# cvg/limap

Hardware: AMD Instinct MI355X
Metric: 3D line candidates scored/sec (100 views x 500 segs per GPU, matched topk=10) (higher is better)
Workload: dtype f64

## Files before the change

### limap_amd/csrc/lt_api.cpp

```cpp

#include "lt_host.h"

using namespace lt;
using namespace lt_impl;

namespace lt_trace {
typedef int (*push_fn)(const char *);
typedef int (*pop_fn)(void);
static push_fn g_push = nullptr;
static pop_fn g_pop = nullptr;
static void init_once() {
  static bool done = false;
  if (done) return;
  done = true;
  const char *sw = getenv("LT_ROCTX");
  if (sw && sw[0] == '0') return;
  const char *libs[] = {"librocprofiler-sdk-roctx.so.1", "librocprofiler-sdk-roctx.so", "libroctx64.so.4", "libroctx64.so"};
  for (const char *l : libs) {
    void *h = dlopen(l, RTLD_LAZY | RTLD_GLOBAL);
    if (!h) continue;
    g_push = (push_fn)dlsym(h, "roctxRangePushA");
    g_pop = (pop_fn)dlsym(h, "roctxRangePop");
    if (g_push && g_pop) return;
    g_push = nullptr;
// ... 204 lines not shown

double now_ms() {
  return std::chrono::duration<double, std::milli>(std::chrono::steady_clock::now().time_since_epoch()).count();
}

}

namespace lt_impl {

double multiplier(double score_th) { return 1.0 / std::sqrt(-std::log(score_th) * 2.0); }

LinkCfg2 make_l2(const lt_config &c) {
  LinkCfg2 l;
  l.score_th = c.l2_score_th; l.th_angle = c.l2_th_angle; l.th_overlap = c.l2_th_overlap;
  l.th_smartoverlap = c.l2_th_smartoverlap; l.th_smartangle = c.l2_th_smartangle;
  l.th_perp = c.l2_th_perp; l.th_innerseg = c.l2_th_innerseg;
  l.mult = multiplier(c.l2_score_th);
  l.use_angle = c.l2_use_angle; l.use_overlap = c.l2_use_overlap; l.use_smartangle = c.l2_use_smartangle;
  l.use_perp = c.l2_use_perp; l.use_innerseg = c.l2_use_innerseg; l.pad_ = 0;
  return l;
}
LinkCfg3 make_l3(const lt_config &c) {
  LinkCfg3 l;
  l.score_th = c.l3_score_th; l.th_angle = c.l3_th_angle; l.th_overlap = c.l3_th_overlap;
  l.th_smartoverlap = c.l3_th_smartoverlap; l.th_smartangle = c.l3_th_smartangle;
  l.th_perp = c.l3_th_perp; l.th_innerseg = c.l3_th_innerseg; l.th_scaleinv = c.l3_th_scaleinv;
  l.mult = multiplier(c.l3_score_th);
  l.use_angle = c.l3_use_angle; l.use_overlap = c.l3_use_overlap; l.use_smartangle = c.l3_use_smartangle;
  l.use_perp = c.l3_use_perp; l.use_innerseg = c.l3_use_innerseg; l.use_scaleinv = c.l3_use_scaleinv;
  return l;
}

GenCfg make_gen(const lt_ctx *ctx) {
  const lt_config &c = ctx->cfg;
  GenCfg g;
  g.min_length_2d = c.min_length_2d; g.angle_th = c.line_tri_angle_threshold; g.iou_th = c.IoU_threshold;
  g.sens_th = c.sensitivity_threshold; g.var2d = c.var2d;
  for (int k = 0; k < 3; ++k) { g.lo[k] = ctx->lo[k]; g.hi[k] = ctx->hi[k]; }
  g.use_ranges = ctx->ranges_on; g.use_endpoints = c.use_endpoints_triangulation;
  g.disable_algebraic = c.disable_algebraic_triangulation;
  g.force_undecided = test_switch("LT_TEST_NO_FAST_GATES") != nullptr;
  if (c.use_vp && !c.disable_vp_triangulation) g.force_undecided = 1;
  double th = c.line_tri_angle_threshold;
  if (th > 1e-3 && th < 89.0) {
    double s = std::sin(th * kPi / 180.0);
    g.sin_lo = s * (1.0 - 1e-7);
    g.sin_hi = s * (1.0 + 1e-7);
  } else {
    g.sin_lo = -1.0;
    g.sin_hi = 1e300;
  }
  {
    const double ths = c.sensitivity_threshold;
    if (ths > 1e-3 && ths < 89.0) {
      const double sn = std::sin(ths * kPi / 180.0);
      g.sens_lo = sn * (1.0 - 1e-7);
      g.sens_hi = sn * (1.0 + 1e-7);
      g.sens_lo2 = g.sens_lo * g.sens_lo * (1.0 - 1e-9);
      g.sens_hi2 = g.sens_hi * g.sens_hi * (1.0 + 1e-9);
    } else {
      g.sens_lo = -1.0;
      g.sens_hi = 1e300;
      g.sens_lo2 = -1.0;
      g.sens_hi2 = 1e300;
    }
    if (test_switch("LT_TEST_NO_FAST_GATES")) {
      g.sens_lo2 = -1.0;
      g.sens_hi2 = 1e300;
    }
  }
  const double L = c.min_length_2d;
  if (L > 0.0) {
    g.len_lo2 = L * L * (1.0 - 1e-12);
    g.len_hi2 = L * L * (1.0 + 1e-12);
  } else if (L == 0.0) {
    g.len_lo2 = g.len_hi2 = 0.0;
  } else {
    g.len_lo2 = g.len_hi2 = -1.0;
  }
  return g;
}

ScoreCfg make_score(const lt_ctx *ctx) {
  ScoreCfg s;
  s.l2 = make_l2(ctx->cfg);
  s.l3 = make_l3(ctx->cfg);
  s.l3.use_angle = 1; s.l3.use_overlap = 0; s.l3.use_perp = 0; s.l3.use_innerseg = 0; s.l3.use_scaleinv = 1;
  double th = s.l3.th_angle * (1.0 + 1e-6) + 1e-6;
  s.cos_guard = (th < 90.0) ? std::cos(th * kPi / 180.0) : -1.0;
  if (test_switch("LT_TEST_NO_SCORE_GUARDS")) s.cos_guard = -1.0;
  s.fullscore_th = ctx->cfg.fullscore_th;
  s.max_valid_conns = ctx->cfg.max_valid_conns;
  auto band = [](double th, double *lo, double *hi) -> bool {
    if (!(th >= 1e-3 && th <= 0.999)) {
      *lo = -1.0;
      *hi = 1e300;
      return false;
    }
    const double q = std::sqrt(-2.0 * std::log(th));
    *lo = q * (1.0 - 1e-9);
    *hi = q * (1.0 + 1e-9);
    return true;
  };
  const bool b3 = band(s.l3.score_th, &s.q3_lo, &s.q3_hi), b2 = band(s.l2.score_th, &s.q2_lo, &s.q2_hi);
  const bool pos = s.l3.th_angle > 0.0 && s.l3.th_scaleinv > 0.0 && s.l2.th_angle > 0.0 && s.l2.th_perp > 0.0 &&
                   s.l2.th_smartangle > 0.0 && s.l2.th_smartangle <= s.l2.th_angle && s.l2.th_smartoverlap > s.l2.th_overlap;
  s.fast = (b3 && b2 && pos && !s.l2.use_innerseg && !test_switch("LT_TEST_PAIR_SCORE_TERMS")) ? 1 : 0;
  return s;
}

int bits_for(long long n) {
  int b = 1;
  while (b < 32 && (1ll << b) < n) ++b;
  return b;
}

int init_common(lt_ctx *ctx, int n_img, const int32_t *img_ids, const int64_t *seg_off_in,
                const std::vector<int> &perm) {
  ctx->n_img = n_img;
  ctx->img_ids.resize(n_img);
  ctx->id2idx.clear();
  ctx->seg_off.assign(n_img + 1, 0);
  for (int i = 0; i < n_img; ++i) {
    ctx->img_ids[i] = img_ids[perm[i]];
    if (ctx->id2idx.count(ctx->img_ids[i])) return fail(ctx, LT_ERR_ARGUMENT, "duplicate image id in Init");
    ctx->id2idx[ctx->img_ids[i]] = i;
    long long m = seg_off_in[perm[i] + 1] - seg_off_in[perm[i]];
    if (m < 0) return fail(ctx, LT_ERR_ARGUMENT, "seg_off must be non-decreasing");
    if (m > 65535) return fail(ctx, LT_ERR_ARGUMENT, "more than 65535 lines in one image (uint16 line ids, util/types.h:16)");
    ctx->seg_off[i + 1] = ctx->seg_off[i] + m;
  }
  ctx->G = ctx->seg_off[n_img];
  if (ctx->G >= (1ll << 32) - 1) return fail(ctx, LT_ERR_ARGUMENT, "too many nodes (>= 2^32-1)");
  ctx->h_node_img.resize(ctx->G);
  for (int i = 0; i < n_img; ++i)
    for (long long g = ctx->seg_off[i]; g < ctx->seg_off[i + 1]; ++g) ctx->h_node_img[g] = i;
  ctx->triangulated.assign(n_img, 0);
  ctx->neighbors.assign(n_img, {});
  lt_host::host_block_release(ctx->best_c_blk);
  ctx->best_c_blk = lt_host::host_block_acquire(sizeof(Cand) * (size_t)std::max<long long>(ctx->G, 1));
  ctx->best_c = (Cand *)ctx->best_c_blk.p;
  if (!ctx->best_c) return fail(ctx, LT_ERR_RUNTIME, "out of host memory for the per-node results");
  ctx->best_c_set.assign(n_img, 0);
  ctx->best_score.assign(ctx->G, 0.0);
  ctx->best_src2.assign(2 * ctx->G, 0);
  ctx->n_tris.assign(ctx->G, 0);
  ctx->has_best.assign(ctx->G, 0);
  ctx->valid_edges.reset(ctx->G);
  ctx->dbg_pool.clear(); ctx->dbg_off.assign((size_t)ctx->G, 0); ctx->dbg_cnt.assign((size_t)ctx->G, 0);
  ctx->vp_ready = false;
  ctx->pts_ready = false; ctx->sfm_given = false; ctx->pts_dirty = false;
  ctx->h_seg_pts.clear(); ctx->h_seg_pt_off.clear(); ctx->h_sfm_ids.clear(); ctx->h_sfm_xyz.clear();
  ctx->tracks.clear();
  ctx->tracks_done = false;
  ctx->job_mode = 0;
  ctx->job_imgs.clear(); ctx->job_nbs.clear(); ctx->job_order.clear();
  ctx->h_m_off.assign(1, 0); ctx->h_m_pairs.clear(); ctx->streamed_ints = 0;
  ctx->h_c_off.clear(); ctx->h_ovf_off.clear(); ctx->h_line0.clear(); ctx->h_ovf.clear();
  ctx->rows_sorted = true;
  ctx->uploaded = ctx->ran = ctx->downloaded = false;
  return LT_OK;
}

int build_invariants(lt_ctx *ctx, const double *hk = nullptr, const double *hq = nullptr, const double *ht = nullptr,
                     const double *hs = nullptr, bool sync = true) {
  hipStream_t st = ctx->stream;
  ENSURE(ctx, ctx->d_cams, sizeof(Cam) * (size_t)std::max(ctx->n_img, 1));
  ENSURE(ctx, ctx->d_segs, sizeof(Seg) * (size_t)std::max<long long>(ctx->G, 1));
  ENSURE(ctx, ctx->d_seg_off, sizeof(long long) * (size_t)(ctx->n_img + 1));
  ENSURE(ctx, ctx->d_node_img, sizeof(int) * (size_t)std::max<long long>(ctx->G, 1));
  HIPCHK(ctx, hipMemcpyAsync(ctx->d_seg_off.p, ctx->seg_off.data(), sizeof(long long) * (ctx->n_img + 1),
                             hipMemcpyHostToDevice, st));
  if (ctx->G > 0)
    HIPCHK(ctx, hipMemcpyAsync(ctx->d_node_img.p, ctx->h_node_img.data(), sizeof(int) * ctx->G,
                               hipMemcpyHostToDevice, st));
  launch_build_cams(st, ctx->n_img, ctx->d_kvec.as<double>(), ctx->d_qvec.as<double>(), ctx->d_tvec.as<double>(),
                    ctx->d_cams.as<Cam>());
  ENSURE(ctx, ctx->d_seg_gates, seg_gate_bytes() * (size_t)std::max<long long>(ctx->G, 1));
  launch_build_segs(st, ctx->G, ctx->n_img, ctx->d_seg_off.as<long long>(), ctx->d_segs_raw.as<double>(),
                    ctx->cfg.add_halfpix ? 0.5 : 0.0, ctx->d_cams.as<Cam>(), ctx->d_segs.as<Seg>(), ctx->d_seg_gates.p);
  HIPCHK(ctx, hipGetLastError());
  if (sync) HIPCHK(ctx, hipStreamSynchronize(st));
  {
    const int n = ctx->n_img;
    std::vector<double> k(4 * (size_t)n), q(4 * (size_t)n), t(3 * (size_t)n);
    if (hk && hq && ht && hs) {
      std::memcpy(k.data(), hk, 32 * (size_t)n);
      std::memcpy(q.data(), hq, 32 * (size_t)n);
      std::memcpy(t.data(), ht, 24 * (size_t)n);
      std::vector<double>().swap(ctx->h_segs);
      ctx->h_segs_ptr = hs;
      ctx->h_segs_add = ctx->cfg.add_halfpix ? 0.5 : 0.0;
    } else {
      ctx->h_segs.assign(4 * (size_t)ctx->G, 0.0);
      if (n > 0) {
        HIPCHK(ctx, hipMemcpy(k.data(), ctx->d_kvec.p, 32 * (size_t)n, hipMemcpyDeviceToHost));
        HIPCHK(ctx, hipMemcpy(q.data(), ctx->d_qvec.p, 32 * (size_t)n, hipMemcpyDeviceToHost));
        HIPCHK(ctx, hipMemcpy(t.data(), ctx->d_tvec.p, 24 * (size_t)n, hipMemcpyDeviceToHost));
      }
      if (ctx->G > 0)
        HIPCHK(ctx, hipMemcpy(ctx->h_segs.data(), ctx->d_segs_raw.p, 32 * (size_t)ctx->G, hipMemcpyDeviceToHost));
    }
    if (!(hk && hq && ht && hs)) {
      ctx->h_segs_ptr = ctx->h_segs.data();
      ctx->h_segs_add = ctx->cfg.add_halfpix ? 0.5 : 0.0;
    }
    ctx->h_cams.resize(n);
    for (int i = 0; i < n; ++i) cam_build(&k[4 * i], &q[4 * i], &t[3 * i], &ctx->h_cams[i]);
  }
  ctx->inited = true;
  return LT_OK;
}

void build_job_tables(lt_ctx *ctx) {
  const int n_img = ctx->n_img;
  ctx->h_nb_off.assign(n_img + 1, 0);
  std::vector<int> job_pos(n_img, -1);
  for (size_t j = 0; j < ctx->job_imgs.size(); ++j) job_pos[ctx->job_imgs[j]] = (int)j;
  ctx->h_blk_img.clear(); ctx->h_blk_nb.clear(); ctx->h_blk_slot.clear(); ctx->h_blk_order.clear();
  ctx->max_nb = 1;
  for (int i = 0; i < n_img; ++i) {
    ctx->h_nb_off[i] = (long long)ctx->h_blk_img.size();
    int j = job_pos[i];
    if (j < 0) continue;
    const auto &nbs = ctx->job_nbs[j];
    ctx->max_nb = std::max(ctx->max_nb, (int)nbs.size());
    for (size_t k = 0; k < nbs.size(); ++k) {
      ctx->h_blk_img.push_back(i);
      ctx->h_blk_nb.push_back(nbs[k]);
      ctx->h_blk_slot.push_back((int)k);
      ctx->h_blk_order.push_back(ctx->job_order[j][k]);
    }
  }
  ctx->h_nb_off[n_img] = (long long)ctx->h_blk_img.size();
  ctx->n_blk = (int)ctx->h_blk_img.size();
  ctx->h_blk_line_base.assign(ctx->n_blk + 1, 0);
  ctx->max_nb_segs = 0;
  ctx->max_own_segs = 0;
  for (int b = 0; b < ctx->n_blk; ++b) {
    int i1 = ctx->h_blk_img[b];
    int i2 = ctx->h_blk_nb[b];
    ctx->max_nb_segs = std::max(ctx->max_nb_segs, (int)(ctx->seg_off[i2 + 1] - ctx->seg_off[i2]));
    ctx->max_own_segs = std::max(ctx->max_own_segs, (int)(ctx->seg_off[i1 + 1] - ctx->seg_off[i1]));
    ctx->h_blk_line_base[b + 1] = ctx->h_blk_line_base[b] + (ctx->seg_off[i1 + 1] - ctx->seg_off[i1]) + 1;
  }
}

}

extern "C" {

void lt_config_default(lt_config *c) {
  std::memset(c, 0, sizeof(*c));
  c->min_length_2d = 20.0; c->line_tri_angle_threshold = 5.0; c->IoU_threshold = 0.1;
  c->sensitivity_threshold = 70.0; c->var2d = 2.0;
  c->fullscore_th = 1.0; c->max_valid_conns = 1000; c->min_num_outer_edges = 1;
  c->merging_strategy = 0; c->num_outliers_aggregator = 2;
  c->l2_score_th = 0.5; c->l2_th_angle = 8.0; c->l2_th_overlap = 0.1; c->l2_th_smartoverlap = 0.2;
  c->l2_th_smartangle = 1.0; c->l2_th_perp = 5.0; c->l2_th_innerseg = 5.0;
  c->l2_use_angle = 1; c->l2_use_overlap = 1; c->l2_use_smartangle = 1; c->l2_use_perp = 1; c->l2_use_innerseg = 0;
  c->l3_score_th = 0.5; c->l3_th_angle = 10.0; c->l3_th_overlap = 0.01; c->l3_th_smartoverlap = 0.1;
  c->l3_th_smartangle = 1.0; c->l3_th_perp = 0.02; c->l3_th_innerseg = 0.02; c->l3_th_scaleinv = 0.01;
  c->l3_use_angle = 1; c->l3_use_overlap = 1; c->l3_use_smartangle = 1; c->l3_use_perp = 0;
  c->l3_use_innerseg = 1; c->l3_use_scaleinv = 0;
}

int lt_abi_version(void) { return 2; }
uint64_t lt_sizeof_config(void) { return (uint64_t)sizeof(lt_config); }

lt_ctx *lt_create(const lt_config *cfg, int device) {
  int n_dev = 0;
  hipError_t e = hipGetDeviceCount(&n_dev);
  if (e != hipSuccess || n_dev <= 0) {
    std::fprintf(stderr, "limap_amd: no HIP device available (%s); this backend has no CPU fallback\n",
                 hipGetErrorString(e));
    return nullptr;
  }
  if (device < 0 || device >= n_dev) {
    std::fprintf(stderr, "limap_amd: device %d out of range (%d devices)\n", device, n_dev);
    return nullptr;
  }
  if (hipSetDevice(device) != hipSuccess) return nullptr;
  lt_ctx *ctx = new lt_ctx();
  ctx->cfg = *cfg;
  ctx->device = device;
  if (!lt_host::stream_set_acquire(device, &ctx->stream, ctx->ev)) {
    if (hipStreamCreateWithFlags(&ctx->stream, hipStreamNonBlocking) != hipSuccess) {
      delete ctx;
      return nullptr;
    }
    for (auto &ev : ctx->ev) (void)hipEventCreate(&ev);
  }
  ctx->pool_stream = ctx->stream;
  ctx->h_pinned_blk = lt_host::host_block_acquire(4096);
  ctx->h_pinned = ctx->h_pinned_blk.pinned ? (long long *)ctx->h_pinned_blk.p : nullptr;
  return ctx;
}

void lt_destroy(lt_ctx *ctx) {
  if (!ctx) return;
  (void)finish_run(ctx);
  (void)hipSetDevice(ctx->device);
  (void)hipStreamSynchronize(ctx->stream);
  DevBuf *bufs[] = {&ctx->d_kvec, &ctx->d_qvec, &ctx->d_tvec, &ctx->d_segs_raw, &ctx->d_cams, &ctx->d_segs,
                    &ctx->d_seg_off, &ctx->d_node_img, &ctx->d_nb_off, &ctx->d_blk_img, &ctx->d_blk_nb,
                    &ctx->d_blk_slot, &ctx->d_blk_order, &ctx->d_m_off, &ctx->d_m_pairs, &ctx->d_c_stream, &ctx->d_ovf, &ctx->d_rowdesc, &ctx->d_pairs,
                    &ctx->d_keys, &ctx->d_rows, &ctx->d_row_blk, &ctx->d_skeys, &ctx->d_srows, &ctx->d_sort_tmp,
                    &ctx->d_conn_off, &ctx->d_st_c, &ctx->d_st_l, &ctx->d_flags, &ctx->d_pos, &ctx->d_scan_tmp,
                    &ctx->d_item_off, &ctx->d_masks, &ctx->d_mask_cnt, &ctx->d_mask_pos, &ctx->d_cand, &ctx->d_hcand, &ctx->d_hlite,
                    &ctx->d_rm_line, &ctx->d_rm_act, &ctx->d_rm_edges, &ctx->d_rm_cnt,
                    &ctx->d_lite, &ctx->d_tri_off, &ctx->d_score, &ctx->d_best_idx, &ctx->d_edge_flag,
                    &ctx->d_nvalid, &ctx->d_edge_off, &ctx->d_edges, &ctx->d_best_c, &ctx->d_best_score,
                    &ctx->d_best_src, &ctx->d_ntris, &ctx->d_err, &ctx->d_blk_line_base, &ctx->d_cnt_bl,
                    &ctx->d_st_key, &ctx->d_wave_count, &ctx->d_wave_pos, &ctx->d_ntris_u, &ctx->d_cand_node,
                    &ctx->d_pair_counter, &ctx->d_result3, &ctx->d_tile_order, &ctx->d_scan_status, &ctx->d_perm, &ctx->d_rng, &ctx->d_chunks, &ctx->d_cand_meta, &ctx->d_st_row, &ctx->d_surv_count, &ctx->d_seg_gates, &ctx->d_blkrec, &ctx->d_seg_vp, &ctx->d_seg_has_vp, &ctx->d_base_bl, &ctx->d_blk_chunk_off, &ctx->d_needed, &ctx->d_seg_pts, &ctx->d_seg_pt_off, &ctx->d_sfm_xyz,
                    &ctx->d_place_perm, &ctx->d_ex_rec, &ctx->d_ex_ent, &ctx->d_node_rec, &ctx->d_ex_z, &ctx->d_tile_list, &ctx->d_tail_keys, &ctx->d_tail_skeys, &ctx->d_tail_sims, &ctx->d_tail_mark,
                    &ctx->d_tail_pos, &ctx->d_tail_recs, &ctx->d_tail_nodes, &ctx->d_tail_tmp, &ctx->d_tail_keep,
                    &ctx->d_tail_kpos, &ctx->d_sp_slots, &ctx->d_sp_cnt, &ctx->d_sp_ovf, &ctx->d_sp_pairs, &ctx->d_sp_desc,
                    &ctx->d_run_len, &ctx->d_slot_row0, &ctx->d_blk_nruns, &ctx->d_ln_flag, &ctx->d_blk_surv, &ctx->d_blk_rnd0,
                    &ctx->d_round_count};
  lt_host::host_block_release(ctx->h_pinned_blk);
  if (ctx->tail_pend.active) lt_host::host_block_release(ctx->tail_pend.hb);
  if (ctx->ev_tail) (void)hipEventDestroy(ctx->ev_tail);
  lt_host::host_block_release(ctx->best_c_blk);
  lt_host::host_block_release(ctx->init_blk);
  for (DevBuf *b : bufs) b->release();
  for (auto &e : ctx->ev_b)
    if (e) (void)hipEventDestroy(e);
  for (auto &e : ctx->ev_end)
    if (e) (void)hipEventDestroy(e);
  if (ctx->pool_stream) (void)hipStreamSynchronize(ctx->pool_stream);
  if (!(ctx->pool_stream && lt_host::stream_set_release(ctx->device, ctx->pool_stream, ctx->ev))) {
    for (auto &ev : ctx->ev)
      if (ev) (void)hipEventDestroy(ev);
    if (ctx->pool_stream) (void)hipStreamDestroy(ctx->pool_stream);
  }
  delete ctx;
}

const char *lt_last_error(lt_ctx *ctx) { return ctx ? ctx->err.c_str() : "null context"; }

int lt_set_stream(lt_ctx *ctx, void *hip_stream) {
  LT_FINISH(ctx);
  HIPCHK(ctx, hipStreamSynchronize(ctx->stream));
  if (hip_stream) {
    ctx->stream = reinterpret_cast<hipStream_t>(hip_stream);
    ctx->own_stream = false;
  } else {
    if (!ctx->pool_stream) HIPCHK(ctx, hipStreamCreateWithFlags(&ctx->pool_stream, hipStreamNonBlocking));
    ctx->stream = ctx->pool_stream;
    ctx->own_stream = true;
  }
  return LT_OK;
}

int lt_set_ranges(lt_ctx *ctx, const double lo[3], const double hi[3]) {
  ctx->ranges_on = true;
  for (int k = 0; k < 3; ++k) { ctx->lo[k] = lo[k]; ctx->hi[k] = hi[k]; }
  return LT_OK;
}
int lt_unset_ranges(lt_ctx *ctx) {
  ctx->ranges_on = false;
  return LT_OK;
}

int lt_init(lt_ctx *ctx, int n_img, const int32_t *img_ids, const double *kvec, const double *qvec,
            const double *tvec, const int64_t *seg_off, const double *segs) {
  LT_FINISH(ctx);
  HIPCHK(ctx, hipSetDevice(ctx->device));
  if (n_img < 0) return fail(ctx, LT_ERR_ARGUMENT, "n_img < 0");
  lt_host::SpinPool::get(lt_host::row_workers()).wake();
  std::vector<int> perm(n_img);
  for (int i = 0; i < n_img; ++i) perm[i] = i;
  std::stable_sort(perm.begin(), perm.end(), [&](int a, int b) { return img_ids[a] < img_ids[b]; });
  static const bool init_trace = getenv("LT_TAIL_TRACE") != nullptr;
  double tl = now_ms();
  auto lap = [&](const char *what) {
    if (!init_trace) return;
    double t = now_ms();
    std::fprintf(stderr, "[init] %-18s %.3f ms\n", what, t - tl);
    tl = t;
  };
  int rc = init_common(ctx, n_img, img_ids, seg_off, perm);
  if (rc) return rc;
  lap("init_common");
  const size_t nI = (size_t)n_img, nG = (size_t)ctx->G;
  const size_t o_q = 4 * nI, o_t = 8 * nI, o_s = 11 * nI + (nI & 1), n_dbl = o_s + 4 * nG;
  if (ctx->init_blk.p) {
    HIPCHK(ctx, hipStreamSynchronize(ctx->stream));
    lt_host::host_block_release(ctx->init_blk);
    ctx->init_blk = lt_host::HostBlock{};
  }
  ctx->init_blk = lt_host::host_block_acquire(8 * std::max<size_t>(n_dbl, 1));
  if (!ctx->init_blk.p) return fail(ctx, LT_ERR_RUNTIME, "out of host memory for the scene");
  double *k = (double *)ctx->init_blk.p, *q = k + o_q, *t = k + o_t, *s = k + o_s;
  for (int i = 0; i < n_img; ++i) {
    int p = perm[i];
    std::memcpy(&k[4 * i], kvec + 4 * p, 32);
    std::memcpy(&q[4 * i], qvec + 4 * p, 32);
    std::memcpy(&t[3 * i], tvec + 3 * p, 24);
    long long m = seg_off[p + 1] - seg_off[p];
    if (m > 0) std::memcpy(&s[4 * ctx->seg_off[i]], segs + 4 * seg_off[p], (size_t)m * 32);
  }
  lap("gather");
  {
    hipStream_t st = ctx->stream;
    ENSURE(ctx, ctx->d_kvec, 32 * std::max<size_t>(nI, 1)); ENSURE(ctx, ctx->d_qvec, 32 * std::max<size_t>(nI, 1));
    ENSURE(ctx, ctx->d_tvec, 24 * std::max<size_t>(nI, 1)); ENSURE(ctx, ctx->d_segs_raw, 32 * std::max<size_t>(nG, 1));
    if (nI > 0) {
      HIPCHK(ctx, hipMemcpyAsync(ctx->d_kvec.p, k, 32 * nI, hipMemcpyHostToDevice, st));
      HIPCHK(ctx, hipMemcpyAsync(ctx->d_qvec.p, q, 32 * nI, hipMemcpyHostToDevice, st));
      HIPCHK(ctx, hipMemcpyAsync(ctx->d_tvec.p, t, 24 * nI, hipMemcpyHostToDevice, st));
    }
    if (nG > 0) HIPCHK(ctx, hipMemcpyAsync(ctx->d_segs_raw.p, s, 32 * nG, hipMemcpyHostToDevice, st));
  }
  lap("upload");
  rc = build_invariants(ctx, k, q, t, s, !ctx->init_blk.pinned);
  lap("build_invariants");
  return rc;
}

int lt_init_vp(lt_ctx *ctx, int n_img, const int32_t *img_ids, const int64_t *label_off, const int32_t *labels,
               const int64_t *vp_off, const double *vps) {
  LT_FINISH(ctx);
  if (!ctx->inited) return fail(ctx, LT_ERR_STATE, "InitVPResults before Init");
  HIPCHK(ctx, hipSetDevice(ctx->device));
  std::vector<double> vp(3 * (size_t)std::max<long long>(ctx->G, 1), 0.0);
  std::vector<unsigned char> has((size_t)std::max<long long>(ctx->G, 1), 0);
  for (int i = 0; i < n_img; ++i) {
    auto it = ctx->id2idx.find(img_ids[i]);
    if (it == ctx->id2idx.end()) return fail(ctx, LT_ERR_ARGUMENT, "InitVPResults: unknown image id " + std::to_string(img_ids[i]));
    const int idx = it->second;
    const long long M = ctx->seg_off[idx + 1] - ctx->seg_off[idx];
    const long long nl = label_off[i + 1] - label_off[i], nv = vp_off[i + 1] - vp_off[i];
    if (nl != M) return fail(ctx, LT_ERR_ARGUMENT, "InitVPResults: " + std::to_string(nl) + " labels for image " +
                                                       std::to_string(img_ids[i]) + " with " + std::to_string(M) + " lines");
    for (long long l = 0; l < M; ++l) {
      const int lab = labels[label_off[i] + l];
      if (lab < 0) continue;
      if (lab >= nv) return fail(ctx, LT_ERR_ARGUMENT, "InitVPResults: VP label out of range");
      const long long g = ctx->seg_off[idx] + l;
      has[(size_t)g] = 1;
      for (int k = 0; k < 3; ++k) vp[3 * (size_t)g + k] = vps[3 * (vp_off[i] + lab) + k];
    }
  }
  int rc;
  if ((rc = upload_vec(ctx, ctx->d_seg_vp, vp))) return rc;
  if ((rc = upload_vec(ctx, ctx->d_seg_has_vp, has))) return rc;
  HIPCHK(ctx, hipStreamSynchronize(ctx->stream));
  ctx->vp_ready = true;
  return LT_OK;
}

int lt_set_bipartites(lt_ctx *ctx, int n_img, const int32_t *img_ids, const int64_t *pt_off, const int32_t *pt_ids,
                      const double *pt_xy, const int32_t *pt_p3d, const int64_t *line_off, const int64_t *lp_off,
                      const int32_t *lp_ptids) {
  LT_FINISH(ctx);
  if (!ctx->inited) return fail(ctx, LT_ERR_STATE, "SetBipartites2d before Init");
  HIPCHK(ctx, hipSetDevice(ctx->device));
  struct SegPointH { int p3d_id, sfm; double x, y; };
  static_assert(sizeof(SegPointH) == 24, "SegPoint layout");
  if (seg_point_bytes() != sizeof(SegPointH)) return fail(ctx, LT_ERR_RUNTIME, "SegPoint layout mismatch");
  std::vector<std::vector<SegPointH>> per_seg((size_t)std::max<long long>(ctx->G, 1));
  for (int i = 0; i < n_img; ++i) {
    auto it = ctx->id2idx.find(img_ids[i]);
    if (it == ctx->id2idx.end()) return fail(ctx, LT_ERR_ARGUMENT, "SetBipartites2d: unknown image id " + std::to_string(img_ids[i]));
    const int idx = it->second;
    const long long M = ctx->seg_off[idx + 1] - ctx->seg_off[idx];
    if (line_off[i + 1] - line_off[i] != M)
      return fail(ctx, LT_ERR_ARGUMENT, "SetBipartites2d: image " + std::to_string(img_ids[i]) + " has " + std::to_string(M) +
                                            " lines, the bipartite lists " + std::to_string(line_off[i + 1] - line_off[i]));
    std::unordered_map<int, long long> row;
    for (long long k = pt_off[i]; k < pt_off[i + 1]; ++k) row[pt_ids[k]] = k;
    for (long long l = 0; l < M; ++l) {
      const long long L = line_off[i] + l;
      std::vector<int> ids(lp_ptids + lp_off[L], lp_ptids + lp_off[L + 1]);
      std::sort(ids.begin(), ids.end());
      ids.erase(std::unique(ids.begin(), ids.end()), ids.end());
      std::map<int, SegPointH> by3d;
      for (int pid : ids) {
        auto r = row.find(pid);
        if (r == row.end()) return fail(ctx, LT_ERR_ARGUMENT, "SetBipartites2d: a line refers to an unknown point id");
        SegPointH sp{pt_p3d[r->second], -1, pt_xy[2 * r->second], pt_xy[2 * r->second + 1]};
        by3d.insert({sp.p3d_id, sp});
      }
      auto &dst = per_seg[(size_t)(ctx->seg_off[idx] + l)];
      dst.clear();
      for (auto &kv : by3d) dst.push_back(kv.second);
    }
  }
  ctx->h_seg_pt_off.assign((size_t)ctx->G + 1, 0);
  ctx->h_seg_pts.clear();
  for (long long g = 0; g < ctx->G; ++g) {
    ctx->h_seg_pt_off[(size_t)g] = (long long)(ctx->h_seg_pts.size() / 3);
    for (auto &sp : per_seg[(size_t)g]) {
      double packed[3];
      std::memcpy(packed, &sp, 24);
      ctx->h_seg_pts.insert(ctx->h_seg_pts.end(), packed, packed + 3);
    }
  }
  ctx->h_seg_pt_off[(size_t)ctx->G] = (long long)(ctx->h_seg_pts.size() / 3);
  ctx->max_seg_pts = 0;
  for (long long g = 0; g < ctx->G; ++g)
    ctx->max_seg_pts = std::max(ctx->max_seg_pts, ctx->h_seg_pt_off[(size_t)g + 1] - ctx->h_seg_pt_off[(size_t)g]);
  ctx->pts_ready = true;
  ctx->pts_dirty = true;
  ctx->uploaded = ctx->ran = false;
  return LT_OK;
}

int lt_set_sfm_points(lt_ctx *ctx, int64_t n, const int32_t *ids, const double *xyz) {
  LT_FINISH(ctx);
  ctx->h_sfm_ids.assign(ids, ids + n);
  ctx->h_sfm_xyz.assign(xyz, xyz + 3 * n);
  ctx->sfm_given = n > 0;
  ctx->pts_dirty = true;
  ctx->uploaded = ctx->ran = false;
  return LT_OK;
}

extern "C++" {
namespace lt_impl {
int upload_points(lt_ctx *ctx) {
  if (!ctx->pts_ready || !ctx->pts_dirty) return LT_OK;
  std::vector<double> pts = ctx->h_seg_pts;
  if (ctx->sfm_given) {
    std::unordered_map<int, int> where;
    for (size_t k = 0; k < ctx->h_sfm_ids.size(); ++k) where[ctx->h_sfm_ids[k]] = (int)k;
    for (size_t e = 0; e + 3 <= pts.size(); e += 3) {
      int head[2];
      std::memcpy(head, &pts[e], 8);
      auto it = where.find(head[0]);
      head[1] = it == where.end() ? -1 : it->second;
      std::memcpy(&pts[e], head, 8);
    }
  }
  if (pts.empty()) pts.assign(3, 0.0);
  int rc;
  if ((rc = upload_vec(ctx, ctx->d_seg_pts, pts))) return rc;
  if ((rc = upload_vec(ctx, ctx->d_seg_pt_off, ctx->h_seg_pt_off))) return rc;
  std::vector<double> xyz = ctx->h_sfm_xyz;
  if (xyz.empty()) xyz.assign(3, 0.0);
  if ((rc = upload_vec(ctx, ctx->d_sfm_xyz, xyz))) return rc;
  HIPCHK(ctx, hipStreamSynchronize(ctx->stream));
  ctx->pts_dirty = false;
  return LT_OK;
}
}
}

int lt_init_device(lt_ctx *ctx, int n_img, const int32_t *img_ids, const void *d_kvec, const void *d_qvec,
                   const void *d_tvec, const int64_t *seg_off, const void *d_segs) {
  LT_FINISH(ctx);
  HIPCHK(ctx, hipSetDevice(ctx->device));
  std::vector<int> perm(n_img);
  for (int i = 0; i < n_img; ++i) {
    perm[i] = i;
    if (i > 0 && img_ids[i] <= img_ids[i - 1])
      return fail(ctx, LT_ERR_ARGUMENT, "lt_init_device needs strictly ascending image ids");
  }
  int rc = init_common(ctx, n_img, img_ids, seg_off, perm);
  if (rc) return rc;
  hipStream_t st = ctx->stream;
  ENSURE(ctx, ctx->d_kvec, 32 * (size_t)std::max(n_img, 1));
  ENSURE(ctx, ctx->d_qvec, 32 * (size_t)std::max(n_img, 1));
  ENSURE(ctx, ctx->d_tvec, 24 * (size_t)std::max(n_img, 1));
  ENSURE(ctx, ctx->d_segs_raw, 32 * (size_t)std::max<long long>(ctx->G, 1));
  if (n_img > 0) {
    HIPCHK(ctx, hipMemcpyAsync(ctx->d_kvec.p, d_kvec, 32 * (size_t)n_img, hipMemcpyDeviceToDevice, st));
    HIPCHK(ctx, hipMemcpyAsync(ctx->d_qvec.p, d_qvec, 32 * (size_t)n_img, hipMemcpyDeviceToDevice, st));
    HIPCHK(ctx, hipMemcpyAsync(ctx->d_tvec.p, d_tvec, 24 * (size_t)n_img, hipMemcpyDeviceToDevice, st));
  }
  if (ctx->G > 0)
    HIPCHK(ctx, hipMemcpyAsync(ctx->d_segs_raw.p, d_segs, 32 * (size_t)ctx->G, hipMemcpyDeviceToDevice, st));
  return build_invariants(ctx);
}

int lt_refresh_scene_device(lt_ctx *ctx, const void *d_kvec, const void *d_qvec, const void *d_tvec,
                            const void *d_segs) {
  if (!ctx->inited) return fail(ctx, LT_ERR_STATE, "lt_refresh_scene_device before Init");
  HIPCHK(ctx, hipSetDevice(ctx->device));
  hipStream_t st = ctx->stream;
  const int n_img = ctx->n_img;
  if (n_img > 0) {
    HIPCHK(ctx, hipMemcpyAsync(ctx->d_kvec.p, d_kvec, 32 * (size_t)n_img, hipMemcpyDeviceToDevice, st));
    HIPCHK(ctx, hipMemcpyAsync(ctx->d_qvec.p, d_qvec, 32 * (size_t)n_img, hipMemcpyDeviceToDevice, st));
    HIPCHK(ctx, hipMemcpyAsync(ctx->d_tvec.p, d_tvec, 24 * (size_t)n_img, hipMemcpyDeviceToDevice, st));
  }
  if (ctx->G > 0)
    HIPCHK(ctx, hipMemcpyAsync(ctx->d_segs_raw.p, d_segs, 32 * (size_t)ctx->G, hipMemcpyDeviceToDevice, st));
  launch_build_cams(st, n_img, ctx->d_kvec.as<double>(), ctx->d_qvec.as<double>(), ctx->d_tvec.as<double>(),
                    ctx->d_cams.as<Cam>());
  ENSURE(ctx, ctx->d_seg_gates, seg_gate_bytes() * (size_t)std::max<long long>(ctx->G, 1));
  launch_build_segs(st, ctx->G, n_img, ctx->d_seg_off.as<long long>(), ctx->d_segs_raw.as<double>(),
                    ctx->cfg.add_halfpix ? 0.5 : 0.0, ctx->d_cams.as<Cam>(), ctx->d_segs.as<Seg>(), ctx->d_seg_gates.p);
  HIPCHK(ctx, hipGetLastError());
  ctx->ran = false;
  return LT_OK;
}

int lt_set_scene_chunks(lt_ctx *ctx, int n_chunks, const int32_t *img_begin, const void *const *d_kvec,
                        const void *const *d_qvec, const void *const *d_tvec, const void *const *d_segs) {
  LT_FINISH(ctx);
  if (!ctx->inited) return fail(ctx, LT_ERR_STATE, "lt_set_scene_chunks before Init");
  if (n_chunks <= 0 || img_begin[0] != 0) return fail(ctx, LT_ERR_ARGUMENT, "chunks must start at image 0");
  HIPCHK(ctx, hipSetDevice(ctx->device));
  std::vector<SceneChunk> ch(n_chunks);
  for (int c = 0; c < n_chunks; ++c) {
    if (img_begin[c] < 0 || img_begin[c] > ctx->n_img || (c > 0 && img_begin[c] < img_begin[c - 1]))
      return fail(ctx, LT_ERR_ARGUMENT, "chunk image ranges must be ascending and inside the scene");
    ch[c].k = (const double *)d_kvec[c]; ch[c].q = (const double *)d_qvec[c]; ch[c].t = (const double *)d_tvec[c];
    ch[c].s = (const double *)d_segs[c];
    ch[c].img_begin = img_begin[c];
    ch[c].seg_begin = ctx->seg_off[img_begin[c]];
    ch[c].pad_ = 0;
  }
  ENSURE(ctx, ctx->d_chunks, sizeof(SceneChunk) * (size_t)n_chunks);
  HIPCHK(ctx, hipMemcpy(ctx->d_chunks.p, ch.data(), sizeof(SceneChunk) * (size_t)n_chunks, hipMemcpyHostToDevice));
  ctx->n_chunks = n_chunks;
  return LT_OK;
}

int lt_refresh_scene_chunks(lt_ctx *ctx) {
  if (!ctx->inited || ctx->n_chunks <= 0) return fail(ctx, LT_ERR_STATE, "lt_refresh_scene_chunks before lt_set_scene_chunks");
  HIPCHK(ctx, hipSetDevice(ctx->device));
  const bool listed = ctx->uploaded && ctx->n_needed > 0;
  launch_build_scene_chunked(ctx->stream, ctx->n_img, ctx->G, ctx->n_chunks, ctx->d_chunks.as<SceneChunk>(),
                             ctx->d_seg_off.as<long long>(), ctx->cfg.add_halfpix ? 0.5 : 0.0, ctx->d_cams.as<Cam>(),
                             ctx->d_segs.as<Seg>(), listed ? ctx->d_needed.as<int>() : nullptr, ctx->n_needed,
                             ctx->max_needed_segs, ctx->d_seg_gates.p);
  HIPCHK(ctx, hipGetLastError());
  ctx->ran = false;
  return LT_OK;
}

}
```

### limap_amd/csrc/lt_api_run.cpp

```cpp
#include "lt_host.h"

using namespace lt;
using namespace lt_impl;

extern "C" {

int lt_upload(lt_ctx *ctx) {
  LT_RANGE("lt_upload (match rows + job tables -> HBM)");
  LT_FINISH(ctx);
  if (!ctx->inited) return fail(ctx, LT_ERR_STATE, "upload before Init");
  if (ctx->uploaded) return LT_OK;
  HIPCHK(ctx, hipSetDevice(ctx->device));
  double t0 = now_ms();
  build_job_tables(ctx);
  ctx->blk_vorder_ok = false;
  int rc;
  {
    std::vector<char> need((size_t)std::max(ctx->n_img, 1), 0);
    for (size_t j = 0; j < ctx->job_imgs.size(); ++j) {
      need[(size_t)ctx->job_imgs[j]] = 1;
      for (int nb : ctx->job_nbs[j]) need[(size_t)nb] = 1;
    }
    std::vector<int> list;
    ctx->max_needed_segs = 0;
    for (int i = 0; i < ctx->n_img; ++i)
      if (need[(size_t)i]) {
        list.push_back(i);
        ctx->max_needed_segs = std::max(ctx->max_needed_segs, ctx->seg_off[i + 1] - ctx->seg_off[i]);
      }
    ctx->n_needed = (int)list.size();
    if (list.empty()) list.push_back(0);
    if ((rc = upload_vec(ctx, ctx->d_needed, list))) return rc;
  }
  if ((rc = upload_vec(ctx, ctx->d_nb_off, ctx->h_nb_off))) return rc;
  if ((rc = upload_vec(ctx, ctx->d_blk_img, ctx->h_blk_img))) return rc;
  if ((rc = upload_vec(ctx, ctx->d_blk_nb, ctx->h_blk_nb))) return rc;
  if ((rc = upload_vec(ctx, ctx->d_blk_slot, ctx->h_blk_slot))) return rc;
  if ((rc = upload_vec(ctx, ctx->d_blk_order, ctx->h_blk_order))) return rc;
  if ((rc = upload_vec(ctx, ctx->d_blk_line_base, ctx->h_blk_line_base))) return rc;
  if (ctx->job_mode == 1) {
    std::vector<long long> call_first_blk(ctx->job_imgs.size() + 1, 0);
    for (size_t j = 0; j < ctx->job_imgs.size(); ++j) call_first_blk[j + 1] = call_first_blk[j] + (long long)ctx->job_nbs[j].size();
    std::vector<int> job_pos(ctx->n_img, -1);
    for (size_t j = 0; j < ctx->job_imgs.size(); ++j) job_pos[ctx->job_imgs[j]] = (int)j;
    std::vector<long long> m_off(ctx->n_blk + 1, 0);
    std::vector<lt::RowDesc> desc((size_t)std::max(ctx->n_blk, 1));
    {
      long long b = 0;
      for (int i = 0; i < ctx->n_img; ++i) {
        int j = job_pos[i];
        if (j < 0) continue;
        for (size_t k = 0; k < ctx->job_nbs[j].size(); ++k, ++b) {
          long long cb = call_first_blk[j] + (long long)k;
          const long long n = ctx->h_m_off[cb + 1] - ctx->h_m_off[cb];
          m_off[b + 1] = m_off[b] + n;
          desc[(size_t)b] = lt::RowDesc{ctx->h_c_off[(size_t)cb], ctx->h_ovf_off[(size_t)cb], m_off[b], (int)n, ctx->h_line0[(size_t)cb]};
        }
      }
    }
    ctx->P = m_off[ctx->n_blk];
    ctx->n_conn = ctx->P;
    ctx->max_rows = 0;
    for (int bq = 0; bq < ctx->n_blk; ++bq) ctx->max_rows = std::max(ctx->max_rows, m_off[bq + 1] - m_off[bq]);
    if (ctx->P >= (1ll << 32) - 1) return fail(ctx, LT_ERR_ARGUMENT, "too many match rows in one batch (>= 2^32-1)");
    ENSURE(ctx, ctx->d_m_pairs, sizeof(int) * (size_t)std::max<long long>(ctx->P, 1));
    const size_t total_w = ctx->h_m_pairs.size();
    if (sizeof(int) * std::max<size_t>(total_w, 1) > ctx->d_c_stream.cap) {
      HIPCHK(ctx, hipStreamSynchronize(ctx->stream));
      ctx->streamed_ints = 0;
      ENSURE(ctx, ctx->d_c_stream, sizeof(int) * std::max<size_t>(total_w, 1));
    }
    {
      const size_t sent = std::min(ctx->streamed_ints, total_w);
      if (total_w > sent)
        HIPCHK(ctx, hipMemcpyAsync(ctx->d_c_stream.as<int>() + sent, ctx->h_m_pairs.data() + sent, sizeof(int) * (total_w - sent),
                                   hipMemcpyHostToDevice, ctx->stream));
      ctx->streamed_ints = total_w;
    }
    if ((rc = upload_vec(ctx, ctx->d_ovf, ctx->h_ovf))) return rc;
    if ((rc = upload_vec(ctx, ctx->d_rowdesc, desc))) return rc;
    const bool extras_cfg = (ctx->cfg.use_vp && !ctx->cfg.disable_vp_triangulation) ||
                            (ctx->pts_ready && (!ctx->cfg.disable_many_points_triangulation || !ctx->cfg.disable_one_point_triangulation));
    bool try_ln = ctx->rows_sorted && ctx->n_blk > 0 && ctx->P > 0 && ctx->max_nb_segs <= 1024 && !extras_cfg &&
                  !test_switch("LT_GEN_ROW_SLOTS") && !test_switch("LT_GEN_NO_LDS_TABLE");
    for (size_t cb = 0; try_ln && cb < ctx->h_ovf_off.size(); ++cb)
      if (ctx->h_ovf_off[cb] >= 0) try_ln = false;
    ctx->rows_ln = false;
    ctx->ln_slots = 0;
    if (try_ln) {
      ctx->ln_slots = gen_slots_ln(ctx->max_own_segs);
      const size_t n_entries = (size_t)std::max<long long>(ctx->h_blk_line_base[ctx->n_blk], 1);
      ENSURE(ctx, ctx->d_run_len, 4 * n_entries);
      ENSURE(ctx, ctx->d_base_bl, 4 * n_entries);
      ENSURE(ctx, ctx->d_slot_row0, 4 * (size_t)ctx->n_blk * (size_t)ctx->ln_slots);
      ENSURE(ctx, ctx->d_blk_nruns, 4 * (size_t)ctx->n_blk);
      ENSURE(ctx, ctx->d_ln_flag, 4);
      HIPCHK(ctx, hipMemsetAsync(ctx->d_ln_flag.p, 0, 4, ctx->stream));
      launch_rows_ln(ctx->stream, ctx->n_blk, ctx->ln_slots, ctx->d_rowdesc.p, ctx->d_c_stream.as<unsigned>(),
                     ctx->d_blk_line_base.as<long long>(), ctx->d_base_bl.as<unsigned>(), ctx->d_blk_nruns.as<int>(),
                     ctx->d_run_len.as<unsigned>(), ctx->d_slot_row0.as<unsigned>(), ctx->d_m_pairs.as<unsigned short>(),
                     ctx->d_ln_flag.as<int>());
      std::vector<unsigned> rnd0((size_t)ctx->n_blk + 1, 0u);
      for (int bq = 0; bq < ctx->n_blk; ++bq) rnd0[(size_t)bq + 1] = rnd0[(size_t)bq] + (unsigned)((m_off[bq + 1] - m_off[bq] + 63) / 64);
      ctx->n_round_slots = (long long)rnd0[(size_t)ctx->n_blk];
      if ((rc = upload_vec(ctx, ctx->d_blk_rnd0, rnd0))) return rc;
      int flag = 0;
      HIPCHK(ctx, hipMemcpyAsync(&flag, ctx->d_ln_flag.p, 4, hipMemcpyDeviceToHost, ctx->stream));
      HIPCHK(ctx, hipStreamSynchronize(ctx->stream));
      ctx->rows_ln = flag == 0;
    }
    if (!ctx->rows_ln)
      launch_expand_rows(ctx->stream, ctx->n_blk, ctx->d_rowdesc.p, ctx->d_c_stream.as<unsigned>(), ctx->d_ovf.as<unsigned>(),
                         ctx->d_m_pairs.as<unsigned>());
    if ((rc = upload_vec(ctx, ctx->d_m_off, m_off))) return rc;
    {
      std::vector<int> vo((size_t)std::max(ctx->n_blk, 1), 0);
      for (int b = 0; b < ctx->n_blk; ++b) vo[(size_t)b] = b;
      std::stable_sort(vo.begin(), vo.begin() + ctx->n_blk, [&](int x, int y) {
        return ctx->h_blk_nb[(size_t)x] != ctx->h_blk_nb[(size_t)y] ? ctx->h_blk_nb[(size_t)x] < ctx->h_blk_nb[(size_t)y]
                                                                    : ctx->h_blk_img[(size_t)x] < ctx->h_blk_img[(size_t)y];
      });
      if ((rc = upload_vec(ctx, ctx->d_blk_vorder, vo))) return rc;
      ctx->blk_vorder_ok = true;
    }
    ENSURE(ctx, ctx->d_blkrec, blk_rec_bytes() * (size_t)std::max(ctx->n_blk, 1));
    launch_build_blk(ctx->stream, ctx->n_blk, ctx->d_m_off.as<long long>(), ctx->d_blk_img.as<int>(),
                     ctx->d_blk_nb.as<int>(), ctx->d_blk_slot.as<int>(), ctx->d_seg_off.as<long long>(),
                     ctx->d_blk_line_base.as<long long>(), ctx->d_blkrec.p);
  } else if (ctx->job_mode == 2) {
    ctx->h_item_off.assign(ctx->G + 1, 0);
    std::vector<int> blk_chunk_off((size_t)std::max(ctx->n_blk, 1), 0);
    ctx->max_chunks = 1;
    long long items = 0, conns = 0;
    for (int i = 0; i < ctx->n_img; ++i) {
      long long per_node = 0, conn_node = 0;
      for (long long b = ctx->h_nb_off[i]; b < ctx->h_nb_off[i + 1]; ++b) {
        int i2 = ctx->h_blk_nb[b];
        long long M2 = ctx->seg_off[i2 + 1] - ctx->seg_off[i2];
        blk_chunk_off[(size_t)b] = (int)per_node;
        ctx->max_chunks = std::max(ctx->max_chunks, (int)((M2 + 63) / 64));
        per_node += (M2 + 63) / 64;
        conn_node += M2;
      }
      for (long long g = ctx->seg_off[i]; g < ctx->seg_off[i + 1]; ++g) {
        ctx->h_item_off[g] = items;
        items += per_node;
        conns += conn_node;
      }
    }
    ctx->h_item_off[ctx->G] = items;
    ctx->P = items;
    ctx->n_conn = conns;
    if ((rc = upload_vec(ctx, ctx->d_item_off, ctx->h_item_off))) return rc;
    if ((rc = upload_vec(ctx, ctx->d_blk_chunk_off, blk_chunk_off))) return rc;
  } else {
    ctx->P = 0;
    ctx->n_conn = 0;
  }
  HIPCHK(ctx, hipStreamSynchronize(ctx->stream));
  ctx->uploaded = true;
  ctx->ran = false;
  ctx->timers[8] = now_ms() - t0;
  return LT_OK;
}

extern "C++" {
namespace lt_impl {
int finish_run(lt_ctx *ctx) {
  LT_RANGE("lt_sync (end of run: result scalars, event timings)");
  if (!ctx->run_pending) return LT_OK;
  ctx->run_pending = false;
  HIPCHK(ctx, hipSetDevice(ctx->device));
  hipEvent_t *ev = ctx->pend_set ? ctx->ev_b : ctx->ev;
  long long *hp = ctx->h_pinned ? ctx->h_pinned + 8 * ctx->pend_set : nullptr;
  int derr = 0;
  if (hp) {
    HIPCHK(ctx, hipEventSynchronize(ctx->pend_ev_end));
    derr = (int)hp[1];
    ctx->stat_pairs_eval = hp[2];
    ctx->C_last = ctx->pend_count_on_device ? hp[0] : ctx->pend_C;
  } else {
    HIPCHK(ctx, hipStreamSynchronize(ctx->stream));
    HIPCHK(ctx, hipMemcpy(&derr, ctx->d_err.p, sizeof(int), hipMemcpyDeviceToHost));
    unsigned long long pe = 0;
    ctx->C_last = ctx->pend_C;
    if (ctx->pend_count_on_device)
      HIPCHK(ctx, hipMemcpy(&ctx->C_last, ctx->d_tri_off.as<long long>() + ctx->G, 8, hipMemcpyDeviceToHost));
    if (ctx->C_last > 0) HIPCHK(ctx, hipMemcpy(&pe, ctx->d_pair_counter.p, 8, hipMemcpyDeviceToHost));
    ctx->stat_pairs_eval = (long long)pe;
  }
  ctx->stat_survivors = -1;
  if (derr == 5) {
    if (ctx->ex_retry_depth > 0 || !ctx->ex_staged_set[ctx->pend_set])
      return fail(ctx, LT_ERR_RUNTIME, "internal: candidate staging overflow outside the one-pass exhaustive mode");
    ctx->ex_two_pass = true;
    if (hp && hp[3] > 0 && ctx->n_conn > 0)
      ctx->ex_frac = 1.4 * (double)hp[3] * (double)ex_regions() / (double)ctx->n_conn;
    if (ctx->in_run_async) return LT_OK;
    ctx->ex_retry_depth = 1;
    int rc2 = lt_run_device_async(ctx);
    if (!rc2) rc2 = finish_run(ctx);
    ctx->ex_retry_depth = 0;
    return rc2;
  }
  if (derr == 8) {
    if (ctx->score_two_kernels)
      return fail(ctx, LT_ERR_RUNTIME, "internal: device flag 8 outside the one-kernel scoring form");
    ctx->score_two_kernels = true;
    if (ctx->in_run_async) return LT_OK;
    const int depth = ctx->ex_retry_depth;
    ctx->ex_retry_depth = depth + 1;
    int rc2 = lt_run_device_async(ctx);
    if (!rc2) rc2 = finish_run(ctx);
    ctx->ex_retry_depth = depth;
    return rc2;
  }
  if (derr == 7) {
    if (ctx->ex_retry_depth > 1)
      return fail(ctx, LT_ERR_RUNTIME, "internal: pair chunk overflow outside the split scoring form");
    ctx->score_fused = true;
    if (ctx->in_run_async) return LT_OK;
    const int depth = ctx->ex_retry_depth;
    ctx->ex_retry_depth = depth + 1;
    int rc2 = lt_run_device_async(ctx);
    if (!rc2) rc2 = finish_run(ctx);
    ctx->ex_retry_depth = depth;
    return rc2;
  }
  ctx->timers[17] = ctx->timers[18] = 0.0;
  if (hp && ctx->ex_staged_set[ctx->pend_set]) {
    ctx->timers[17] = (double)hp[3] * (double)ex_regions();
    ctx->timers[18] = (double)ctx->ex_region_cap * (double)ex_regions();
  }
  if (ctx->job_mode == 2 && derr == 0 && ctx->n_conn > 0) {
    if (hp && ctx->ex_staged_set[ctx->pend_set])
      ctx->ex_frac = std::max(1.4 * (double)hp[3] * (double)ex_regions() / (double)ctx->n_conn, 1e-4);
    else if (ctx->ex_frac <= 0.0)
      ctx->ex_frac = std::max(2.2 * (double)ctx->C_last / (double)ctx->n_conn, 1e-4);
    ctx->ex_two_pass = false;
  }
  if (derr == 4) return fail(ctx, LT_ERR_RUNTIME, "internal: the scan of the node counts did not complete");
  if (derr == 3)
    return fail(ctx, LT_ERR_RUNTIME, "more than 65 000 candidates on one connection of the exhaustive mode (16-bit counts)");
  if (derr == 2)
    return fail(ctx, LT_ERR_RUNTIME, "map::at: a point shared by two lines has a point3D_id that is not among the SfM points");
  if (derr != 0) return fail(ctx, LT_ERR_RUNTIME, "IndexError! Out-of-index matches detected on the device");
  float ms;
  ctx->timers[1] = ctx->timers[2] = ctx->timers[7] = 0.0;
  const int eg = ctx->pend_ev_gen_end, ep = ctx->pend_ev_place_end;
  const hipEvent_t e_start = ctx->pend_ev_start ? ctx->pend_ev_start : ev[0];
  const hipEvent_t e_end = hp ? ctx->pend_ev_end : ev[7];
  HIPCHK(ctx, hipEventElapsedTime(&ms, e_start, e_end));
  ctx->timers[0] = ms;
  const bool sampled = ctx->pend_sampled;
  if (sampled) {
  const hipEvent_t kA[4] = {e_start, ev[eg], ev[ep], ev[5]}, kB[4] = {ev[eg], ev[ep], ev[5], e_end};
  const int kT[4] = {3, 4, 5, 6};
  for (int k = 0; k < 4; ++k) {
    HIPCHK(ctx, hipEventElapsedTime(&ms, kA[k], kB[k]));
    ctx->timers[kT[k]] = ms;
  }
  ctx->timers[13] = ctx->timers[14] = ctx->timers[15] = 0.0;
  if (ctx->pend_fine_gen && ctx->job_mode == 1 && ctx->n_blk > 0 && ctx->max_rows > 0) {
    if (hipEventElapsedTime(&ms, ev[8], ev[9]) == hipSuccess) ctx->timers[13] = ms;
    if (hipEventElapsedTime(&ms, ev[9], ev[10]) == hipSuccess) ctx->timers[14] = ms;
  }
  if (ctx->pend_fine_score && ctx->C_last > 0 && hipEventElapsedTime(&ms, ev[11], ev[5]) == hipSuccess) ctx->timers[15] = ms;
  (void)hipGetLastError();
  ++ctx->timer_stage_runs;
  }
  ctx->timers[11] = (double)ctx->stat_pairs_eval;
  for (int k = 0; k < 24; ++k) {
    const bool stage = (k >= 3 && k <= 6) || (k >= 13 && k <= 15);
    if (k != 8 && k != 9 && k != 10 && k != 12 && k != 16 && (sampled || !stage)) ctx->timer_sums[k] += ctx->timers[k];
  }
  ++ctx->timer_runs;
  return LT_OK;
}
}
}
int lt_sync(lt_ctx *ctx) { return finish_run(ctx); }

int lt_run_device_async(lt_ctx *ctx) {
  LT_RANGE("lt_run_device (enqueue: generation, placement, scoring, selection)");
  if (!ctx->uploaded) return fail(ctx, LT_ERR_STATE, "lt_run_device before lt_upload");
  if (!ctx->h_pinned) LT_FINISH(ctx);
  ctx->shard_keys = ctx->shard_own_keys = -1;
  if (ctx->inited && !ctx->best_c_set.empty())
    for (int idx : ctx->job_imgs)
      if (ctx->best_c_set[(size_t)idx] == 1) {
        ctx->best_c_set[(size_t)idx] = 0;
        for (long long g = ctx->seg_off[idx]; g < ctx->seg_off[idx + 1]; ++g) {
          if ((size_t)g < ctx->has_best.size()) ctx->has_best[(size_t)g] = 0;
          if ((size_t)g < ctx->valid_edges.cnt.size()) ctx->valid_edges.cnt[(size_t)g] = 0;
        }
      }
  const int set = ctx->run_pending ? (ctx->pend_set ^ 1) : 0;
  if (ctx->h_pinned) std::memset(ctx->h_pinned + 8 * set, 0, 32);
  if (set == 1 && !ctx->ev_b[0])
    for (auto &e : ctx->ev_b) HIPCHK(ctx, hipEventCreate(&e));
  hipEvent_t *ev = set ? ctx->ev_b : ctx->ev;
  long long *hp = ctx->h_pinned ? ctx->h_pinned + 8 * set : nullptr;
  ctx->ex_staged_set[set] = false;
  int sample_n = 8;
  if (const char *e = getenv("LT_TIMER_SAMPLE")) sample_n = std::max(1, atoi(e));
  if (!(ctx->run_pending && hp)) ctx->async_seq = 0;
  const bool sampled = (ctx->async_seq++ % (unsigned)sample_n) == 0u;
  const bool fine_gen = sampled && fine_gen_timers(), fine_score = sampled && fine_timers();
  HIPCHK(ctx, hipSetDevice(ctx->device));
  hipStream_t st = ctx->stream;
  const long long G = ctx->G, P = ctx->P;
  {
    int rcp = upload_points(ctx);
    if (rcp) return rcp;
  }
  GenCfg gcfg = make_gen(ctx);
  if (ctx->pts_ready && (!ctx->cfg.disable_many_points_triangulation || !ctx->cfg.disable_one_point_triangulation))
    gcfg.force_undecided = 1;
  const ScoreCfg scfg = make_score(ctx);
  const bool score_f32 = !test_switch("LT_TEST_SCORE_F64");
  const bool guards_on = scfg.l3.th_scaleinv > 0.0 && scfg.l3.score_th > 0.0 && scfg.l3.score_th < 1.0 &&
                         !test_switch("LT_TEST_NO_SCORE_GUARDS");
  const double guard2 = guards_on ? (scfg.l3.th_scaleinv * (1.0 + 1e-6)) * (scfg.l3.th_scaleinv * (1.0 + 1e-6)) : 1e300;
  ENSURE(ctx, ctx->d_err, sizeof(int));
  ENSURE(ctx, ctx->d_pair_counter, 8);
  ENSURE(ctx, ctx->d_result3, 32);
  ENSURE(ctx, ctx->d_pairs, sizeof(PairRec) * (size_t)std::max(ctx->n_blk, 1));
  ENSURE(ctx, ctx->d_tri_off, sizeof(long long) * (size_t)(G + 1));
  hipEvent_t ev_start = ev[0];
  if (ctx->run_pending && hp && ctx->pend_ev_end && !test_switch("LT_TEST_OWN_START_EVENT")) ev_start = ctx->pend_ev_end;
  else HIPCHK(ctx, hipEventRecord(ev[0], st));
  const int n_status_scan = (int)((G + 1 + 255) / 256) + 1;
  const int n_status = n_status_scan + score3_tile_buckets() * 16 + ex_regions() * 16 + 8 * 16;
  ENSURE(ctx, ctx->d_scan_status, 8 * (size_t)n_status);
  const bool ln_job = ctx->job_mode == 1 && ctx->rows_ln && ctx->rows_sorted;
  if (ln_job) ENSURE(ctx, ctx->d_blk_surv, 4 * (size_t)std::max(ctx->n_blk, 1));
  launch_build_pairs(st, ctx->n_blk, ctx->d_blk_img.as<int>(), ctx->d_blk_nb.as<int>(), ctx->d_cams.as<Cam>(),
                     ctx->d_pairs.as<PairRec>(), ctx->d_err.as<int>(),
                     ctx->d_pair_counter.as<unsigned long long>(), ctx->d_scan_status.as<unsigned long long>(),
                     n_status, ln_job ? ctx->d_blk_surv.as<unsigned>() : nullptr);

  bool node_rec_valid = false;
  long long C_known = -1;
  long long C_bound = 0;
  int ev_gen_end = 3, ev_place_end = 4;
  long long C_run = 0;
  if (ctx->job_mode == 1) {
    const size_t Pn = (size_t)std::max<long long>(P, 1);
    const bool fast = ctx->rows_sorted;
    {
      const bool vp_now = ctx->cfg.use_vp && !ctx->cfg.disable_vp_triangulation;
      const bool pts_now = ctx->pts_ready && (!ctx->cfg.disable_many_points_triangulation || !ctx->cfg.disable_one_point_triangulation);
      if (ctx->rows_ln && (vp_now || pts_now)) {
        launch_expand_rows(st, ctx->n_blk, ctx->d_rowdesc.p, ctx->d_c_stream.as<unsigned>(), ctx->d_ovf.as<unsigned>(),
                           ctx->d_m_pairs.as<unsigned>());
        ctx->rows_ln = false;
      }
    }
    const bool ln = ctx->rows_ln && fast;
    const int ln_slots = ln ? ctx->ln_slots : 0;
    if (ln) ENSURE(ctx, ctx->d_round_count, 4 * (size_t)std::max<long long>(ctx->n_round_slots, 1));
    const long long n_waves = (long long)ctx->n_blk * gen_groups(ctx->max_rows);
    const long long n_slots_all = (long long)ctx->n_blk * (ln ? ln_slots : gen_slots(ctx->max_rows));
    const long long n_entries = ctx->h_blk_line_base[ctx->n_blk];
    const bool vp_on = ctx->cfg.use_vp && !ctx->cfg.disable_vp_triangulation;
    if (vp_on && !ctx->vp_ready) return fail(ctx, LT_ERR_STATE, "use_vp is set but InitVPResults was not called");
    const bool pts_any = ctx->pts_ready && (!ctx->cfg.disable_many_points_triangulation || !ctx->cfg.disable_one_point_triangulation);
    const bool many_on = pts_any && !ctx->cfg.disable_many_points_triangulation;
    const bool one_on = pts_any && !ctx->cfg.disable_one_point_triangulation;
    const bool pts_on = pts_any;
    const bool extras = vp_on || pts_on;
    long long staged_total = -1;
    if (!extras) {
      ENSURE(ctx, ctx->d_st_c, sizeof(CRec) * Pn); ENSURE(ctx, ctx->d_st_l, sizeof(double) * Pn);
      ENSURE(ctx, ctx->d_st_key, 4 * (Pn + 64));
    }
    ENSURE(ctx, ctx->d_wave_count, 4 * (size_t)(n_waves + 1));
    if (extras) ENSURE(ctx, ctx->d_wave_pos, 8 * (size_t)(n_waves + 1));
    const long long *group_base = extras ? ctx->d_wave_pos.as<long long>() : nullptr;
    ENSURE(ctx, ctx->d_ntris_u, 4 * (size_t)(G + 1));
    if (fast) {
      const size_t nb = 4 * (size_t)std::max<long long>(n_entries, 1);
      const void *before = ctx->d_cnt_bl.p;
      ENSURE(ctx, ctx->d_cnt_bl, nb);
      ENSURE(ctx, ctx->d_base_bl, nb);
      if (ctx->d_cnt_bl.p != before || !ctx->cnt_bl_clean || ctx->cnt_bl_bytes != nb) {
        HIPCHK(ctx, hipMemsetAsync(ctx->d_cnt_bl.p, 0, ctx->d_cnt_bl.cap, st));
        ctx->cnt_bl_bytes = nb;
      }
      ctx->cnt_bl_clean = false;
    }
    const bool no_lds_table = test_switch("LT_GEN_NO_LDS_TABLE") != nullptr;
    int lds_segs = (!no_lds_table && ctx->max_nb_segs <= 1024) ? ctx->max_nb_segs : 0;
    int lds_segs1 = (!no_lds_table && ctx->max_own_segs <= 1024) ? ctx->max_own_segs : 0;
    if (lds_segs + lds_segs1 > 1024) lds_segs1 = 0;
    if (ln) {
      lds_segs = std::max(ctx->max_nb_segs, 1);
      lds_segs1 = 0;
    }
    {
      ENSURE(ctx, ctx->d_st_row, 8 * Pn);
      ENSURE(ctx, ctx->d_surv_count, 4 * (size_t)(n_slots_all + 1));
      if (!ctx->d_seg_gates.p) return fail(ctx, LT_ERR_STATE, "segment gate records missing (Init not run?)");
      auto gen = [&](int phase) {
      launch_gen_split(st, ctx->n_blk, ctx->max_rows, gcfg, ctx->d_m_off.as<long long>(), ctx->d_m_pairs.as<int>(),
                       ctx->d_blk_img.as<int>(), ctx->d_blk_nb.as<int>(), ctx->d_blk_slot.as<int>(),
                       ctx->d_seg_off.as<long long>(), ctx->d_cams.as<Cam>(), ctx->d_segs.as<Seg>(),
                       ctx->d_pairs.as<PairRec>(), ctx->d_blk_line_base.as<long long>(), ctx->d_st_c.as<CRec>(),
                       ctx->d_st_l.as<double>(), ctx->d_st_key.as<unsigned>(), ctx->d_wave_count.as<unsigned>(),
                       fast ? ctx->d_cnt_bl.as<unsigned>() : nullptr, lds_segs, lds_segs1, ctx->d_st_row.p,
                       ctx->d_surv_count.as<unsigned>(), G, ctx->d_seg_gates.p, ctx->d_blkrec.p, fine_gen ? &ev[8] : nullptr,
                       vp_on ? ctx->d_seg_vp.as<double>() : nullptr,
                       vp_on ? ctx->d_seg_has_vp.as<unsigned char>() : nullptr,
                       pts_on ? ctx->d_seg_pt_off.as<long long>() : nullptr, pts_on ? ctx->d_seg_pts.p : nullptr,
                       (pts_on && ctx->sfm_given) ? ctx->d_sfm_xyz.as<double>() : nullptr, ctx->d_err.as<int>(),
                       many_on ? 1 : 0, one_on ? 1 : 0, group_base, phase, ln_slots, ctx->d_m_pairs.as<unsigned short>(),
                       ctx->d_run_len.as<unsigned>(), ctx->d_slot_row0.as<unsigned>(), ctx->d_blk_surv.as<unsigned>(),
                       ctx->d_blk_rnd0.as<unsigned>(), ctx->d_round_count.as<unsigned>(),
                       (ctx->blk_vorder_ok && !test_switch("LT_TEST_GATES_IMAGE_MAJOR")) ? ctx->d_blk_vorder.as<int>() : nullptr,
                       test_switch("LT_TEST_TRI_STATIC") ? nullptr
                           : (unsigned *)(ctx->d_scan_status.as<unsigned long long>() + n_status_scan + score3_tile_buckets() * 16 + ex_regions() * 16));
      };
      if (!extras) {
        gen(0);
      } else {
        gen(1);
        HIPCHK(ctx, hipMemsetAsync(ctx->d_wave_count.as<unsigned>() + n_waves, 0, 4, st));
        size_t tmp = scan_temp_bytes_u32_to_i64(n_waves + 1);
        ENSURE(ctx, ctx->d_scan_tmp, std::max<size_t>(tmp, 16));
        if (launch_scan_u32_to_i64(st, ctx->d_scan_tmp.p, tmp, n_waves + 1, ctx->d_wave_count.as<unsigned>(),
                                   ctx->d_wave_pos.as<long long>()) != 0)
          return fail(ctx, LT_ERR_HIP, "rocprim scan failed");
        HIPCHK(ctx, hipMemcpyAsync(&staged_total, ctx->d_wave_pos.as<long long>() + n_waves, 8, hipMemcpyDeviceToHost, st));
        HIPCHK(ctx, hipStreamSynchronize(st));
        if (staged_total >= (1ll << 32) - 1)
          return fail(ctx, LT_ERR_ARGUMENT, "too many candidates in one batch (>= 2^32-1): triangulate the images in smaller batches");
        const size_t Sn = (size_t)std::max<long long>(staged_total, 1);
        ENSURE(ctx, ctx->d_st_c, sizeof(CRec) * Sn); ENSURE(ctx, ctx->d_st_l, sizeof(double) * Sn);
        ENSURE(ctx, ctx->d_st_key, 4 * Sn);
        gen(2);
      }
    }
    bool gen_event_pending = false;
    if (fine_gen && ctx->n_blk > 0 && ctx->max_rows > 0) ev_gen_end = 10;
    else gen_event_pending = true;
    long long *hC = hp;
    long long hC_fallback = 0;
    if (!hC) hC = &hC_fallback;
    if (fast) {
      ENSURE(ctx, ctx->d_node_rec, 16 * (size_t)std::max<long long>(G, 1));
      launch_node_prefix(st, G, ctx->d_node_img.as<int>(), ctx->d_seg_off.as<long long>(),
                         ctx->d_nb_off.as<long long>(), ctx->d_blk_line_base.as<long long>(),
                         ctx->d_cnt_bl.as<unsigned>(), ctx->d_base_bl.as<unsigned>(), ctx->d_ntris_u.as<unsigned>(),
                         ctx->d_tri_off.as<long long>(), ctx->d_scan_status.as<unsigned long long>(),
                         ctx->d_err.as<int>(), ctx->d_node_rec.p);
      node_rec_valid = true;
      ctx->cnt_bl_clean = true;
      const long long bound = P;
      constexpr long long kCountFreeBytes = 48ll << 30;
      const bool perm_bound = !test_switch("LT_TEST_PLACE_COPY");
      const long long per_cand = (perm_bound ? 4 : (long long)(sizeof(CRec) + 8)) + 8 + 4 + 4 + (long long)cand_meta_bytes() +
                                 (long long)score_split_entry_bytes() * 256 / 64;
      if (extras) {
        C_known = staged_total;
      } else if (ctx->h_pinned && bound * per_cand <= kCountFreeBytes && !test_switch("LT_TEST_SYNC_COUNT")) {
        C_known = -1;
        C_bound = bound;
      } else {
        HIPCHK(ctx, hipMemcpyAsync(hC, ctx->d_tri_off.as<long long>() + G, 8, hipMemcpyDeviceToHost, st));
        HIPCHK(ctx, hipStreamSynchronize(st));
        C_known = *hC;
      }
    } else {
      ENSURE(ctx, ctx->d_wave_pos, 8 * (size_t)(n_waves + 1));
      HIPCHK(ctx, hipMemsetAsync(ctx->d_wave_count.as<unsigned>() + n_waves, 0, 4, st));
      size_t tmp = scan_temp_bytes_u32_to_i64(n_waves + 1);
      ENSURE(ctx, ctx->d_scan_tmp, std::max<size_t>(tmp, 16));
      if (launch_scan_u32_to_i64(st, ctx->d_scan_tmp.p, tmp, n_waves + 1, ctx->d_wave_count.as<unsigned>(),
                                 ctx->d_wave_pos.as<long long>()) != 0)
        return fail(ctx, LT_ERR_HIP, "rocprim scan failed");
      HIPCHK(ctx, hipMemcpyAsync(hC, ctx->d_wave_pos.as<long long>() + n_waves, 8, hipMemcpyDeviceToHost, st));
      HIPCHK(ctx, hipStreamSynchronize(st));
      C_known = *hC;
    }
    const bool perm_mode = fast && !test_switch("LT_TEST_PLACE_COPY");
    ctx->perm_mode = perm_mode;
    ctx->compact_valid = !perm_mode;
    if (C_known < 0) {
      const size_t Bn = (size_t)std::max<long long>(C_bound, 1);
      const bool got = (perm_mode ? ctx->d_place_perm.ensure(4 * Bn)
                                  : (ctx->d_cand.ensure(sizeof(CRec) * Bn) && ctx->d_lite.ensure(sizeof(double) * Bn))) &&
                       ctx->d_score.ensure(8 * Bn) && ctx->d_edge_flag.ensure(4 * Bn) && ctx->d_cand_node.ensure(4 * Bn) &&
                       ctx->d_cand_meta.ensure(cand_meta_bytes() * Bn);
      if (!got) {
        (void)hipGetLastError();
        HIPCHK(ctx, hipMemcpyAsync(hC, ctx->d_tri_off.as<long long>() + G, 8, hipMemcpyDeviceToHost, st));
        HIPCHK(ctx, hipStreamSynchronize(st));
        C_known = *hC;
      }
    }
    if (C_known >= 0) C_bound = C_known;
    const size_t Cn = (size_t)std::max<long long>(C_bound, 1);
    if (perm_mode) {
      ENSURE(ctx, ctx->d_place_perm, 4 * Cn);
    } else {
      ENSURE(ctx, ctx->d_cand, sizeof(CRec) * Cn); ENSURE(ctx, ctx->d_lite, sizeof(double) * Cn);
    }
    ENSURE(ctx, ctx->d_score, 8 * Cn); ENSURE(ctx, ctx->d_edge_flag, 4 * Cn); ENSURE(ctx, ctx->d_cand_node, 4 * Cn);
    ctx->cand_cap = (long long)Cn;
    if (fast) {
      launch_place(st, ctx->n_blk, ctx->max_rows, ctx->d_m_off.as<long long>(), ctx->d_blk_img.as<int>(),
                   ctx->d_seg_off.as<long long>(), ctx->d_blk_line_base.as<long long>(),
                   ctx->d_base_bl.as<unsigned>(), ctx->d_wave_count.as<unsigned>(), ctx->d_tri_off.as<long long>(),
                   ctx->d_st_c.as<CRec>(), ctx->d_st_l.as<double>(), ctx->d_st_key.as<unsigned>(),
                   ctx->d_cand.as<CRec>(), ctx->d_lite.as<double>(), ctx->d_cand_node.as<unsigned>(), group_base,
                   perm_mode ? ctx->d_place_perm.as<unsigned>() : nullptr, ctx->d_blk_surv.as<unsigned>(),
                   ctx->d_blk_rnd0.as<unsigned>(), ln ? ctx->d_round_count.as<unsigned>() : nullptr);
    } else {
      ENSURE(ctx, ctx->d_keys, 4 * Cn); ENSURE(ctx, ctx->d_rows, 4 * Cn);
      ENSURE(ctx, ctx->d_skeys, 4 * Cn); ENSURE(ctx, ctx->d_srows, 4 * Cn);
      launch_pack_keys(st, ctx->n_blk, ctx->max_rows, ctx->d_m_off.as<long long>(),
                       ctx->d_wave_count.as<unsigned>(), ctx->d_wave_pos.as<long long>(),
                       ctx->d_st_key.as<unsigned>(), ctx->d_keys.as<unsigned>(), ctx->d_rows.as<unsigned>(), group_base);
      if (C_known > 0) {
        int end_bit = bits_for(G + 1);
        size_t tmp = sort_temp_bytes(C_known, end_bit);
        ENSURE(ctx, ctx->d_sort_tmp, std::max<size_t>(tmp, 16));
        if (launch_sort(st, ctx->d_sort_tmp.p, tmp, C_known, ctx->d_keys.as<unsigned>(), ctx->d_skeys.as<unsigned>(),
                        ctx->d_rows.as<unsigned>(), ctx->d_srows.as<unsigned>(), end_bit) != 0)
          return fail(ctx, LT_ERR_HIP, "rocprim radix sort failed");
      }
      launch_node_offsets(st, C_known, G, ctx->d_skeys.as<unsigned>(), ctx->d_tri_off.as<long long>());
      launch_permute(st, C_known, ctx->d_skeys.as<unsigned>(), ctx->d_srows.as<unsigned>(), ctx->d_st_c.as<CRec>(),
                     ctx->d_st_l.as<double>(), ctx->d_cand.as<CRec>(), ctx->d_lite.as<double>(),
                     ctx->d_cand_node.as<unsigned>());
    }
    if (fine_score && C_bound > 0) ev_place_end = 11;
    else if (sampled) HIPCHK(ctx, hipEventRecord(ev[4], st));
    if (gen_event_pending) ev_gen_end = ev_place_end;
  } else if (ctx->job_mode == 2) {
    ctx->perm_mode = false;
    ctx->compact_valid = true;
    const size_t In = (size_t)std::max<long long>(P, 1);
    const bool vp_on = ctx->cfg.use_vp && !ctx->cfg.disable_vp_triangulation;
    if (vp_on && !ctx->vp_ready) return fail(ctx, LT_ERR_STATE, "use_vp is set but InitVPResults was not called");
    const double *seg_vp = vp_on ? ctx->d_seg_vp.as<double>() : nullptr;
    const unsigned char *seg_has_vp = vp_on ? ctx->d_seg_has_vp.as<unsigned char>() : nullptr;
    const int n_masks = vp_on ? 3 : 1;
    const bool pts_any = ctx->pts_ready && (!ctx->cfg.disable_many_points_triangulation || !ctx->cfg.disable_one_point_triangulation);
    const int many_on = (pts_any && !ctx->cfg.disable_many_points_triangulation) ? 1 : 0;
    const int one_on = (pts_any && !ctx->cfg.disable_one_point_triangulation) ? 1 : 0;
    const double *sfm_xyz = (pts_any && ctx->sfm_given) ? ctx->d_sfm_xyz.as<double>() : nullptr;
    ENSURE(ctx, ctx->d_masks, pts_any ? 128 * In : 8 * (In * n_masks + 1)); ENSURE(ctx, ctx->d_mask_cnt, 4 * (In + 1));
    ENSURE(ctx, ctx->d_mask_pos, 8 * (In + 1));
    const bool plain = !pts_any && !vp_on;
    bool staged = plain && ctx->h_pinned && !ctx->ex_two_pass && P > 0 && !test_switch("LT_TEST_EX_TWO_PASS") &&
                  !test_switch("LT_TEST_EX_PASS1_BLOCK");
    long long ex_cap = 0;
    unsigned region_cap = 0;
    unsigned long long *ex_ctr = ctx->d_scan_status.as<unsigned long long>() + n_status_scan + score3_tile_buckets() * 16;
    if (staged) {
      double frac = ctx->ex_frac > 0.0 ? ctx->ex_frac : 1.0 / 6.0;
      long long slack = 65536;
      if (const char *f = test_switch("LT_TEST_EX_CAP_FRAC")) {
        frac = atof(f);
        slack = 0;
      }
      const long long want = (long long)((double)ctx->n_conn * frac) + slack;
      const long long nreg = ex_regions();
      const long long rc8 = ((want + nreg - 1) / nreg + 63) & ~63ll;
      ex_cap = nreg * rc8;
      if (ex_cap >= (1ll << 32) - 1 || ex_cap * 210 > (64ll << 30)) staged = false;
      else {
        region_cap = (unsigned)rc8;
        const size_t Bn = (size_t)ex_cap;
        const bool got = ctx->d_st_c.ensure(sizeof(CRec) * Bn) && ctx->d_st_l.ensure(sizeof(double) * Bn) &&
                         ctx->d_st_key.ensure(4 * Bn) && ctx->d_place_perm.ensure(4 * Bn) && ctx->d_score.ensure(8 * Bn) &&
                         ctx->d_edge_flag.ensure(4 * Bn) && ctx->d_cand_node.ensure(4 * Bn) &&
                         ctx->d_cand_meta.ensure(cand_meta_bytes() * Bn) && ctx->d_ex_rec.ensure(4 * Bn) &&
                         ctx->d_ex_ent.ensure(8 * Bn) && ctx->d_ex_z.ensure(4 * Bn);
        if (!got) {
          (void)hipGetLastError();
          staged = false;
        }
      }
    }
    ctx->ex_staged_set[set] = staged;
    if (pts_any) {
      launch_gen_exhaustive_pts(st, false, P, gcfg, ctx->d_item_off.as<long long>(), G, ctx->d_node_img.as<int>(),
                                ctx->d_nb_off.as<long long>(), ctx->d_blk_nb.as<int>(), ctx->d_seg_off.as<long long>(),
                                ctx->d_cams.as<Cam>(), ctx->d_segs.as<Seg>(), ctx->d_pairs.as<PairRec>(),
                                ctx->d_masks.as<unsigned short>(), ctx->d_mask_cnt.as<unsigned>(), nullptr, nullptr,
                                nullptr, seg_vp, seg_has_vp, ctx->d_seg_pt_off.as<long long>(), ctx->d_seg_pts.p,
                                sfm_xyz, ctx->d_err.as<int>(), many_on, one_on, ctx->d_blk_chunk_off.as<int>(),
                                ctx->max_nb, ctx->max_chunks, ctx->d_seg_gates.p);
    } else {
      if (plain && !test_switch("LT_TEST_EX_PASS1_BLOCK"))
        launch_gates_exhaustive(st, ctx->n_blk, ctx->max_chunks, P, gcfg, ctx->d_item_off.as<long long>(),
                                ctx->d_blk_img.as<int>(), ctx->d_blk_nb.as<int>(), ctx->d_seg_off.as<long long>(),
                                ctx->d_cams.as<Cam>(), ctx->d_segs.as<Seg>(), ctx->d_pairs.as<PairRec>(),
                                ctx->d_masks.as<unsigned long long>(), ctx->d_blk_chunk_off.as<int>(), ctx->d_seg_gates.p,
                                staged ? ctx->d_ex_ent.as<unsigned long long>() : nullptr, ex_ctr, region_cap,
                                ctx->d_err.as<int>());
      else
      launch_gen_exhaustive(st, false, P, gcfg, ctx->d_item_off.as<long long>(), G, ctx->d_node_img.as<int>(),
                            ctx->d_nb_off.as<long long>(), ctx->d_blk_nb.as<int>(), ctx->d_seg_off.as<long long>(),
                            ctx->d_cams.as<Cam>(), ctx->d_segs.as<Seg>(), ctx->d_pairs.as<PairRec>(),
                            ctx->d_masks.as<unsigned long long>(), nullptr, nullptr, nullptr, seg_vp, seg_has_vp,
                            ctx->d_blk_chunk_off.as<int>(), ctx->max_nb, ctx->max_chunks, ctx->d_seg_gates.p);
      if (staged) {
        HIPCHK(ctx, hipMemsetAsync(ctx->d_masks.p, 0, 8 * In, st));
        launch_tri_exhaustive(st, ctx->d_ex_ent.as<unsigned long long>(), ex_ctr, region_cap, gcfg, P,
                              ctx->d_item_off.as<long long>(), ctx->d_blk_img.as<int>(), ctx->d_blk_nb.as<int>(),
                              ctx->d_nb_off.as<long long>(), ctx->d_seg_off.as<long long>(), ctx->d_cams.as<Cam>(),
                              ctx->d_segs.as<Seg>(), ctx->d_pairs.as<PairRec>(), ctx->d_blk_chunk_off.as<int>(),
                              ctx->d_masks.as<unsigned long long>(), ctx->d_st_c.as<CRec>(), ctx->d_st_l.as<double>(),
                              ctx->d_st_key.as<unsigned>(), ctx->d_ex_z.as<float>());
      }
      if (!plain) launch_popc(st, P, ctx->d_masks.as<unsigned long long>(), ctx->d_mask_cnt.as<unsigned>(), n_masks);
    }
    if (plain) {
      HIPCHK(ctx, hipMemsetAsync(ctx->d_masks.as<unsigned long long>() + P, 0, 8, st));
      size_t tmp = scan_temp_bytes_popc(P + 1);
      ENSURE(ctx, ctx->d_scan_tmp, std::max<size_t>(tmp, 16));
      if (launch_scan_popc(st, ctx->d_scan_tmp.p, tmp, P + 1, ctx->d_masks.as<unsigned long long>(),
                           ctx->d_mask_pos.as<long long>()) != 0)
        return fail(ctx, LT_ERR_HIP, "rocprim scan failed");
    } else {
      HIPCHK(ctx, hipMemsetAsync(ctx->d_mask_cnt.as<unsigned>() + P, 0, 4, st));
      size_t tmp = scan_temp_bytes_u32_to_i64(P + 1);
      ENSURE(ctx, ctx->d_scan_tmp, std::max<size_t>(tmp, 16));
      if (launch_scan_u32_to_i64(st, ctx->d_scan_tmp.p, tmp, P + 1, ctx->d_mask_cnt.as<unsigned>(),
                                 ctx->d_mask_pos.as<long long>()) != 0)
        return fail(ctx, LT_ERR_HIP, "rocprim scan failed");
    }
    if (staged) {
      launch_tri_offsets_ex(st, G, ctx->d_item_off.as<long long>(), ctx->d_mask_pos.as<long long>(), P, -1, ex_cap,
                            ctx->d_tri_off.as<long long>(), ctx->d_err.as<int>());
      if (sampled) HIPCHK(ctx, hipEventRecord(ev[3], st));
      launch_place_exhaustive(st, ex_ctr, region_cap, ctx->d_ex_ent.as<unsigned long long>(),
                              ctx->d_st_key.as<unsigned>(), ctx->d_item_off.as<long long>(),
                              ctx->d_blk_chunk_off.as<int>(), ctx->d_masks.as<unsigned long long>(),
                              ctx->d_mask_pos.as<long long>(), P, ctx->d_tri_off.as<long long>(), G,
                              ctx->d_place_perm.as<unsigned>(), (hp ? hp : ctx->d_result3.as<long long>()) + 3);
      ctx->ex_region_cap = region_cap;
      launch_cand_node(st, G, ctx->d_tri_off.as<long long>(), ctx->d_cand_node.as<unsigned>());
      ctx->perm_mode = true;
      ctx->compact_valid = false;
      ctx->cand_cap = ex_cap;
      C_known = -1;
      C_bound = ex_cap;
      if (sampled) HIPCHK(ctx, hipEventRecord(ev[4], st));
    } else {
    long long total = 0;
    HIPCHK(ctx, hipMemcpyAsync(&total, ctx->d_mask_pos.as<long long>() + P, 8, hipMemcpyDeviceToHost, st));
    HIPCHK(ctx, hipStreamSynchronize(st));
    if (sampled) HIPCHK(ctx, hipEventRecord(ev[3], st));
    const size_t Cn = (size_t)std::max<long long>(total, 1);
    ENSURE(ctx, ctx->d_cand, sizeof(CRec) * Cn); ENSURE(ctx, ctx->d_lite, sizeof(double) * Cn);
    ENSURE(ctx, ctx->d_score, 8 * Cn); ENSURE(ctx, ctx->d_edge_flag, 4 * Cn);
    ctx->cand_cap = (long long)Cn;
    if (pts_any)
      launch_gen_exhaustive_pts(st, true, P, gcfg, ctx->d_item_off.as<long long>(), G, ctx->d_node_img.as<int>(),
                                ctx->d_nb_off.as<long long>(), ctx->d_blk_nb.as<int>(), ctx->d_seg_off.as<long long>(),
                                ctx->d_cams.as<Cam>(), ctx->d_segs.as<Seg>(), ctx->d_pairs.as<PairRec>(),
                                ctx->d_masks.as<unsigned short>(), ctx->d_mask_cnt.as<unsigned>(),
                                ctx->d_mask_pos.as<long long>(), ctx->d_cand.as<CRec>(), ctx->d_lite.as<double>(),
                                seg_vp, seg_has_vp, ctx->d_seg_pt_off.as<long long>(), ctx->d_seg_pts.p, sfm_xyz,
                                ctx->d_err.as<int>(), many_on, one_on, ctx->d_blk_chunk_off.as<int>(), ctx->max_nb,
                                ctx->max_chunks, ctx->d_seg_gates.p);
    else if (!vp_on && !test_switch("LT_TEST_EX_PASS2_BLOCK"))
      launch_fill_exhaustive(st, ctx->n_blk, P, gcfg, ctx->d_item_off.as<long long>(), ctx->d_blk_img.as<int>(),
                             ctx->d_blk_nb.as<int>(), ctx->d_nb_off.as<long long>(), ctx->d_seg_off.as<long long>(),
                             ctx->d_cams.as<Cam>(), ctx->d_segs.as<Seg>(), ctx->d_pairs.as<PairRec>(),
                             ctx->d_masks.as<unsigned long long>(), ctx->d_mask_pos.as<long long>(),
                             ctx->d_cand.as<CRec>(), ctx->d_lite.as<double>(), ctx->d_blk_chunk_off.as<int>());
    else
      launch_gen_exhaustive(st, true, P, gcfg, ctx->d_item_off.as<long long>(), G, ctx->d_node_img.as<int>(),
                            ctx->d_nb_off.as<long long>(), ctx->d_blk_nb.as<int>(), ctx->d_seg_off.as<long long>(),
                            ctx->d_cams.as<Cam>(), ctx->d_segs.as<Seg>(), ctx->d_pairs.as<PairRec>(),
                            ctx->d_masks.as<unsigned long long>(), ctx->d_mask_pos.as<long long>(),
                            ctx->d_cand.as<CRec>(), ctx->d_lite.as<double>(), seg_vp, seg_has_vp,
                            ctx->d_blk_chunk_off.as<int>(), ctx->max_nb, ctx->max_chunks, ctx->d_seg_gates.p);
    launch_tri_offsets_ex(st, G, ctx->d_item_off.as<long long>(), ctx->d_mask_pos.as<long long>(), P, total, -1,
                          ctx->d_tri_off.as<long long>(), ctx->d_err.as<int>());
    ENSURE(ctx, ctx->d_cand_node, 4 * Cn);
    launch_cand_node(st, G, ctx->d_tri_off.as<long long>(), ctx->d_cand_node.as<unsigned>());
    C_known = total;
    C_bound = total;
    if (sampled) HIPCHK(ctx, hipEventRecord(ev[4], st));
    }
  } else {
    ctx->perm_mode = false;
    ctx->compact_valid = true;
    HIPCHK(ctx, hipMemsetAsync(ctx->d_tri_off.p, 0, sizeof(long long) * (size_t)(G + 1), st));
    ENSURE(ctx, ctx->d_cand, sizeof(CRec)); ENSURE(ctx, ctx->d_lite, sizeof(double));
    ENSURE(ctx, ctx->d_score, 8); ENSURE(ctx, ctx->d_edge_flag, 4); ENSURE(ctx, ctx->d_cand_node, 4);
    C_known = 0;
    C_bound = 0;
    for (int k = 3; k <= 4; ++k)
      if (sampled) HIPCHK(ctx, hipEventRecord(ev[k], st));
  }

  if (score3_lds_bytes(ctx->max_nb, score_f32) > 160 * 1024)
    return fail(ctx, LT_ERR_ARGUMENT, "too many neighbours for the scoring kernel's LDS budget");
  {
    if (ctx->h_nb_off[ctx->n_img] >= (1ll << 24))
      return fail(ctx, LT_ERR_ARGUMENT, "too many (image, neighbour) blocks in one batch (>= 2^24)");
    ENSURE(ctx, ctx->d_cand_meta, cand_meta_bytes() * (size_t)std::max<long long>(C_bound, 1));
    ENSURE(ctx, ctx->d_tile_order, 64 * 128);
    const bool tile_classes = !test_switch("LT_TEST_NO_TILE_CLASSES") && ctx->job_mode == 1;
    const unsigned tile_cap = (unsigned)(((std::max<long long>(C_bound, 1) + 63) / 64 + 7) / 8);
    if (tile_classes) ENSURE(ctx, ctx->d_tile_list, 16 * (size_t)tile_cap * (size_t)score3_tile_buckets());
    const bool score_sorted = score_f32 && ctx->job_mode == 2 && !test_switch("LT_TEST_SCORE_UNSORTED");
    if (score_sorted) {
      ENSURE(ctx, ctx->d_perm, 4 * (size_t)std::max<long long>(C_bound, 1));
      ENSURE(ctx, ctx->d_rng, 4 * (size_t)std::max<long long>(C_bound, 1));
    }
    const bool staged_sorted = score_sorted && ctx->perm_mode && ctx->job_mode == 2;
    C_run = C_bound;
    const bool split = score_f32 && !ctx->score_fused && !test_switch("LT_SCORE_FUSED") &&
                       (tile_classes || staged_sorted || test_switch("LT_SCORE_SPLIT"));
    long long sp_chunks = 0;
    int sp_slot_cap = ctx->job_mode == 2 ? 64 : 256;
    if (split) {
      const long long n_tiles_b = (std::max<long long>(C_bound, 1) + 63) / 64;
      sp_chunks = score_split_chunks(std::max<long long>(C_bound, 1));
      if (const char *e = test_switch("LT_TEST_SPLIT_CHUNKS")) sp_chunks = std::max(0, atoi(e));
      if (const char *e = test_switch("LT_TEST_SPLIT_SLOT")) sp_slot_cap = std::max(1, atoi(e));
      ENSURE(ctx, ctx->d_sp_slots, score_split_entry_bytes() * (size_t)sp_slot_cap * (size_t)n_tiles_b);
      ENSURE(ctx, ctx->d_sp_cnt, 4 * (size_t)n_tiles_b);
      ENSURE(ctx, ctx->d_sp_ovf, 4 * (size_t)n_tiles_b);
      ENSURE(ctx, ctx->d_sp_pairs, score_split_chunk_bytes() * (size_t)std::max<long long>(sp_chunks, 1));
      ENSURE(ctx, ctx->d_sp_desc, 8 * (size_t)std::max<long long>(sp_chunks, 1));
    }
    const bool pair_classes = split && tile_classes && !test_switch("LT_TEST_NO_PAIR_CLASSES");
    if (pair_classes) {
      ENSURE(ctx, ctx->d_pc_cnt, 128 * (size_t)score3_tile_buckets());
      ENSURE(ctx, ctx->d_pc_list, 8 * (size_t)tile_cap * (size_t)score3_tile_buckets());
    }
    launch_score3(st, C_bound, G, ctx->d_tri_off.as<long long>(), ctx->d_cand_node.as<unsigned>(), ctx->d_cand_meta.p,
                  ctx->perm_mode ? ctx->d_st_c.as<CRec>() : ctx->d_cand.as<CRec>(), ctx->d_node_img.as<int>(),
                  ctx->d_nb_off.as<long long>(), ctx->d_blk_order.as<int>(), ctx->d_cams.as<Cam>(),
                  ctx->d_score.as<double>(), ctx->d_pair_counter.as<unsigned long long>(), ctx->max_nb, scfg,
                  guard2, fine_score ? ev[11] : nullptr, ctx->d_tile_order.as<unsigned>(), score_f32,
                  (ctx->perm_mode && !staged_sorted) ? ctx->d_place_perm.as<unsigned>()
                                                     : (score_sorted ? ctx->d_perm.as<unsigned>() : nullptr),
                  score_sorted ? ctx->d_rng.p : nullptr, ctx->perm_mode && !staged_sorted,
                  tile_classes ? (unsigned *)(ctx->d_scan_status.as<unsigned long long>() + n_status_scan) : nullptr,
                  tile_classes ? ctx->d_tile_list.as<unsigned>() : nullptr, tile_cap,
                  staged_sorted ? ctx->d_place_perm.as<unsigned>() : nullptr,
                  staged_sorted ? ctx->d_ex_rec.as<unsigned>() : nullptr,
                  staged_sorted ? ctx->d_ex_z.as<float>() : nullptr, ctx->d_err.as<int>(),
                  split ? ctx->d_sp_slots.p : nullptr, sp_slot_cap, ctx->d_sp_cnt.as<unsigned>(),
                  ctx->d_sp_ovf.as<unsigned>(), ctx->d_sp_pairs.p, ctx->d_sp_desc.p, sp_chunks, sampled ? ev[5] : nullptr,
                  node_rec_valid ? ctx->d_node_rec.p : nullptr, pair_classes ? ctx->d_pc_cnt.as<unsigned>() : nullptr,
                  pair_classes ? ctx->d_pc_list.p : nullptr, tile_cap,
                  (((ctx->score_two_kernels || test_switch("LT_SCORE_TWO_KERNELS") || ctx->n_img >= (1 << 18))
                        ? 0 : (test_switch("LT_TEST_Q_LOSE_TILE") ? 2 : 1)) |
                   (test_switch("LT_TEST_DENSE_TABLES") ? 4 : 0) | (test_switch("LT_TEST_DENSE_FEW_ROWS") ? 8 : 0)));
    if (C_bound <= 0 && sampled) HIPCHK(ctx, hipEventRecord(ev[5], st));
  }
  ENSURE(ctx, ctx->d_best_idx, 8 * (size_t)std::max<long long>(G, 1));
  ENSURE(ctx, ctx->d_nvalid, 4 * (size_t)(G + 1));
  ENSURE(ctx, ctx->d_edge_off, 8 * (size_t)(G + 1));
  ENSURE(ctx, ctx->d_best_c, sizeof(Cand) * (size_t)std::max<long long>(G, 1));
  ENSURE(ctx, ctx->d_best_score, 8 * (size_t)std::max<long long>(G, 1));
  ENSURE(ctx, ctx->d_best_src, 8 * (size_t)std::max<long long>(G, 1));
  ENSURE(ctx, ctx->d_ntris, 4 * (size_t)std::max<long long>(G, 1));
  launch_select(st, G, ctx->d_tri_off.as<long long>(), ctx->d_score.as<double>(), scfg.fullscore_th,
                scfg.max_valid_conns, ctx->d_best_idx.as<long long>(), ctx->d_edge_flag.as<unsigned>(),
                ctx->d_nvalid.as<unsigned>(), ctx->perm_mode ? ctx->d_st_c.as<CRec>() : ctx->d_cand.as<CRec>(),
                ctx->perm_mode ? ctx->d_st_l.as<double>() : ctx->d_lite.as<double>(),
                ctx->d_best_c.as<Cand>(), ctx->d_best_score.as<double>(), ctx->d_best_src.as<int>(),
                ctx->d_ntris.as<int>(), ctx->job_mode == 2, ctx->d_err.as<int>(),
                ctx->d_pair_counter.as<unsigned long long>(), hp ? hp : ctx->d_result3.as<long long>(),
                ctx->perm_mode ? ctx->d_place_perm.as<unsigned>() : nullptr);
  if (!hp) HIPCHK(ctx, hipEventRecord(ev[7], st));
  HIPCHK(ctx, hipGetLastError());
  hipEvent_t ev_end = nullptr;
  if (hp) {
    if (!ctx->ev_end[0])
      for (auto &e : ctx->ev_end) HIPCHK(ctx, hipEventCreate(&e));
    ev_end = ctx->ev_end[ctx->run_seq++ % 3u];
    HIPCHK(ctx, hipEventRecord(ev_end, st));
  }
  int rc_prev = LT_OK;
  if (ctx->run_pending) {
    ctx->in_run_async = true;
    rc_prev = finish_run(ctx);
    ctx->in_run_async = false;
  }
  ctx->run_pending = true;
  ctx->pend_ev_start = ev_start;
  ctx->pend_sampled = sampled;
  ctx->pend_ev_end = ev_end;
  ctx->pend_set = set;
  ctx->pend_count_on_device = C_known < 0;
  ctx->pend_fine_gen = fine_gen;
  ctx->pend_fine_score = fine_score;
  ctx->pend_C = C_run;
  ctx->pend_ev_gen_end = ev_gen_end;
  ctx->pend_ev_place_end = ev_place_end;
  ctx->ran = true;
  ctx->downloaded = false;
  ctx->host_view_valid = false;
  return rc_prev;
}

int lt_run_device(lt_ctx *ctx) {
  int rc = lt_run_device_async(ctx);
  if (rc) return rc;
  return finish_run(ctx);
}

extern "C++" {
namespace lt_impl {
void define_best_of_other_images(lt_ctx *ctx) {
  for (int i = 0; i < ctx->n_img; ++i)
    if (!ctx->best_c_set[(size_t)i]) {
      const long long a = ctx->seg_off[i], b = ctx->seg_off[i + 1];
      if (b > a) std::memset((void *)(ctx->best_c + a), 0, sizeof(Cand) * (size_t)(b - a));
      ctx->best_c_set[(size_t)i] = 2;
    }
}
}
}

extern "C++" {
namespace lt_impl {
int materialize_compact(lt_ctx *ctx) {
  if (ctx->host_view_valid) return LT_OK;
  const long long C = ctx->C_last;
  const size_t Cn = (size_t)std::max<long long>(C, 1);
  ENSURE(ctx, ctx->d_hcand, sizeof(Cand) * Cn); ENSURE(ctx, ctx->d_hlite, sizeof(CandLite) * Cn);
  launch_host_view(ctx->stream, C, ctx->perm_mode ? ctx->d_place_perm.as<unsigned>() : nullptr,
                   ctx->perm_mode ? ctx->d_st_c.as<CRec>() : ctx->d_cand.as<CRec>(),
                   ctx->perm_mode ? ctx->d_st_l.as<double>() : ctx->d_lite.as<double>(), ctx->d_hcand.as<Cand>(),
                   ctx->d_hlite.as<CandLite>());
  HIPCHK(ctx, hipStreamSynchronize(ctx->stream));
  ctx->host_view_valid = true;
  return LT_OK;
}
}
}

int lt_download(lt_ctx *ctx) {
  LT_RANGE("lt_download (per-node results -> host)");
  LT_FINISH(ctx);
  if (!ctx->ran) return fail(ctx, LT_ERR_STATE, "lt_download before lt_run_device");
  if (ctx->downloaded) return LT_OK;
  HIPCHK(ctx, hipSetDevice(ctx->device));
  double t0 = now_ms();
  hipStream_t st = ctx->stream;
  const long long G = ctx->G;
  HIPCHK(ctx, hipMemsetAsync(ctx->d_nvalid.as<unsigned>() + G, 0, 4, st));
  {
    size_t tmp = scan_temp_bytes_u32_to_i64(G + 1);
    ENSURE(ctx, ctx->d_scan_tmp, std::max<size_t>(tmp, 16));
    if (launch_scan_u32_to_i64(st, ctx->d_scan_tmp.p, tmp, G + 1, ctx->d_nvalid.as<unsigned>(),
                               ctx->d_edge_off.as<long long>()) != 0)
      return fail(ctx, LT_ERR_HIP, "rocprim scan failed");
  }
  std::vector<long long> tri_off(G + 1), edge_off(G + 1);
  HIPCHK(ctx, hipMemcpyAsync(tri_off.data(), ctx->d_tri_off.p, 8 * (size_t)(G + 1), hipMemcpyDeviceToHost, st));
  HIPCHK(ctx, hipMemcpyAsync(edge_off.data(), ctx->d_edge_off.p, 8 * (size_t)(G + 1), hipMemcpyDeviceToHost, st));
  HIPCHK(ctx, hipStreamSynchronize(st));
  ctx->C = tri_off[G];
  ctx->E = edge_off[G];
  ENSURE(ctx, ctx->d_edges, 8 * (size_t)std::max<long long>(ctx->E, 1));
  launch_edge_fill(st, G, ctx->d_tri_off.as<long long>(), ctx->d_edge_flag.as<unsigned>(),
                   ctx->d_edge_off.as<long long>(), ctx->perm_mode ? ctx->d_st_c.as<CRec>() : ctx->d_cand.as<CRec>(),
                   ctx->d_edges.as<int>(), ctx->perm_mode ? ctx->d_place_perm.as<unsigned>() : nullptr);
  const size_t Gn = (size_t)std::max<long long>(G, 1), En = (size_t)std::max<long long>(ctx->E, 1);
  const size_t o_bc = 0, o_bs = o_bc + sizeof(Cand) * Gn, o_src = o_bs + 8 * Gn, o_nt = o_src + 8 * Gn,
               o_ed = (o_nt + 4 * Gn + 15) / 16 * 16, total = o_ed + 8 * En;
  lt_host::HostBlock hb = lt_host::host_block_acquire(total);
  if (!hb.p) return fail(ctx, LT_ERR_RUNTIME, "out of host memory for the results");
  struct Rel {
    lt_host::HostBlock b;
    ~Rel() { lt_host::host_block_release(b); }
  } rel{hb};
  char *base = (char *)hb.p;
  const Cand *bc = (const Cand *)(base + o_bc);
  const double *bs = (const double *)(base + o_bs);
  const int *bsrc = (const int *)(base + o_src);
  const int *nt = (const int *)(base + o_nt);
  const int *edges = (const int *)(base + o_ed);
  if (G > 0) {
    HIPCHK(ctx, hipMemcpyAsync(base + o_bc, ctx->d_best_c.p, sizeof(Cand) * (size_t)G, hipMemcpyDeviceToHost, st));
    HIPCHK(ctx, hipMemcpyAsync(base + o_bs, ctx->d_best_score.p, 8 * (size_t)G, hipMemcpyDeviceToHost, st));
    HIPCHK(ctx, hipMemcpyAsync(base + o_src, ctx->d_best_src.p, 8 * (size_t)G, hipMemcpyDeviceToHost, st));
    HIPCHK(ctx, hipMemcpyAsync(base + o_nt, ctx->d_ntris.p, 4 * (size_t)G, hipMemcpyDeviceToHost, st));
  }
  if (ctx->E > 0)
    HIPCHK(ctx, hipMemcpyAsync(base + o_ed, ctx->d_edges.p, 8 * (size_t)ctx->E, hipMemcpyDeviceToHost, st));
  HIPCHK(ctx, hipStreamSynchronize(st));
  const long long pool_base = (long long)ctx->valid_edges.pool.size();
  ctx->valid_edges.pool.insert(ctx->valid_edges.pool.end(), edges, edges + 2 * (size_t)ctx->E);
  long long pairs = 0;
  const long long n_job = (long long)ctx->job_imgs.size();
#pragma omp parallel for num_threads(lt::host_threads()) schedule(dynamic, 4) reduction(+ : pairs)
  for (long long j = 0; j < n_job; ++j) {
    const int idx = ctx->job_imgs[(size_t)j];
    ctx->best_c_set[(size_t)idx] = 1;
    for (long long g = ctx->seg_off[idx]; g < ctx->seg_off[idx + 1]; ++g) {
      ctx->n_tris[g] = nt[g];
      pairs += (long long)nt[g] * nt[g];
      ctx->has_best[g] = nt[g] > 0 ? 1 : 0;
      ctx->best_c[g] = bc[g];
      ctx->best_score[g] = bs[g];
      ctx->best_src2[2 * g] = nt[g] > 0 ? ctx->img_ids[bsrc[2 * g]] : 0;
      ctx->best_src2[2 * g + 1] = nt[g] > 0 ? bsrc[2 * g + 1] : 0;
      ctx->valid_edges.off[(size_t)g] = pool_base + 2 * edge_off[g];
      ctx->valid_edges.cnt[(size_t)g] = (int)(2 * (edge_off[g + 1] - edge_off[g]));
    }
  }
  define_best_of_other_images(ctx);
  ctx->stat_pairs = pairs;
  if (ctx->cfg.debug_mode && ctx->C > 0) {
    const long long C = ctx->C;
    {
      int rcm = materialize_compact(ctx);
      if (rcm) return rcm;
    }
    std::vector<Cand> c((size_t)C);
    std::vector<CandLite> l((size_t)C);
    std::vector<double> sc((size_t)C);
    HIPCHK(ctx, hipMemcpy(c.data(), ctx->d_hcand.p, sizeof(Cand) * (size_t)C, hipMemcpyDeviceToHost));
    HIPCHK(ctx, hipMemcpy(l.data(), ctx->d_hlite.p, sizeof(CandLite) * (size_t)C, hipMemcpyDeviceToHost));
    HIPCHK(ctx, hipMemcpy(sc.data(), ctx->d_score.p, 8 * (size_t)C, hipMemcpyDeviceToHost));
    for (long long j = 0; j < n_job; ++j) {
      const int idx = ctx->job_imgs[(size_t)j];
      for (long long g = ctx->seg_off[idx]; g < ctx->seg_off[idx + 1]; ++g) {
        ctx->dbg_off[(size_t)g] = (long long)ctx->dbg_pool.size();
        ctx->dbg_cnt[(size_t)g] = (int)(tri_off[g + 1] - tri_off[g]);
        for (long long t = tri_off[g]; t < tri_off[g + 1]; ++t) {
          lt_ctx::DebugTri r;
          for (int k = 0; k < 3; ++k) { r.line10[k] = c[t].s[k]; r.line10[3 + k] = c[t].e[k]; }
          r.line10[6] = c[t].depth[0]; r.line10[7] = c[t].depth[1]; r.line10[8] = c[t].unc; r.line10[9] = c[t].score3;
          r.score = sc[t];
          r.src2[0] = ctx->img_ids[lite_img(l[t])];
          r.src2[1] = l[t].ng_line;
          ctx->dbg_pool.push_back(r);
        }
      }
    }
  }
  ctx->downloaded = true;
  ctx->timers[9] = now_ms() - t0;
  return LT_OK;
}

int lt_flush(lt_ctx *ctx) {
  int rc;
  if (ctx->job_mode == 0 && !ctx->uploaded) {
    if (!ctx->inited) return fail(ctx, LT_ERR_STATE, "flush before Init");
    ctx->downloaded = true;
    return LT_OK;
  }
  if (!ctx->uploaded && (rc = lt_upload(ctx))) return rc;
  if (!ctx->ran && (rc = lt_run_device(ctx))) return rc;
  if (!ctx->downloaded && (rc = lt_download(ctx))) return rc;
  return LT_OK;
}

}
```

### limap_amd/csrc/lt_ctx.h

```cpp
#pragma once

#include "../../include/limap_amd.h"
#include "lt_device.h"

#include <algorithm>
#include <cstdlib>
#include <cstring>
#include <mutex>
#include <string>
#include <hip/hip_runtime.h>
#include <unordered_map>
#include <vector>

namespace lt_host {
using namespace lt;

void *dev_block_acquire(size_t bytes, size_t *cap);
void dev_block_release(void *p, size_t cap);

struct DevBuf {
  void *p = nullptr;
  size_t cap = 0;
  DevBuf() = default;
  DevBuf(const DevBuf &) = delete;
  DevBuf &operator=(const DevBuf &) = delete;
  ~DevBuf() { release(); }
  void take(DevBuf &o) {
    release();
    p = o.p; cap = o.cap;
    o.p = nullptr; o.cap = 0;
  }
  bool ensure(size_t bytes) {
    if (bytes <= cap) return true;
    if (p) {
      (void)hipDeviceSynchronize();
      dev_block_release(p, cap);
    }
    p = nullptr;
    cap = 0;
    p = dev_block_acquire(bytes + bytes / 8 + 256, &cap);
    return p != nullptr;
  }
  void release() {
    if (p) dev_block_release(p, cap);
    p = nullptr;
    cap = 0;
  }
  template <class T>
  T *as() const { return reinterpret_cast<T *>(p); }
};

struct HostBlock {
  void *p = nullptr;
  size_t bytes = 0;
  bool pinned = false;
};
HostBlock host_block_acquire(size_t bytes);
void host_block_release(HostBlock b);

struct RawInts {
  HostBlock blk;
  size_t n = 0;
  ~RawInts() { host_block_release(blk); }
  RawInts() = default;
  RawInts(const RawInts &) = delete;
  RawInts &operator=(const RawInts &) = delete;
  size_t size() const { return n; }
  size_t capacity() const { return blk.bytes / sizeof(int); }
  int *data() { return (int *)blk.p; }
  const int *data() const { return (const int *)blk.p; }
  void clear() { n = 0; }
  bool grow_to(size_t want) {
    if (want > capacity()) {
      size_t nc = std::max(want, capacity() + capacity() / 2 + 1024);
      HostBlock q = host_block_acquire(nc * sizeof(int));
      if (!q.p) return false;
      if (n) std::memcpy(q.p, blk.p, n * sizeof(int));
      host_block_release(blk);
      blk = q;
    }
    n = want;
    return true;
  }
  bool reserve(size_t want) {
    size_t keep = n;
    if (!grow_to(std::max(want, n))) return false;
    n = keep;
    return true;
  }
};

template <class T>
struct ZeroVec {
  T *p = nullptr;
  size_t n = 0;
  ZeroVec() = default;
  ZeroVec(const ZeroVec &) = delete;
  ZeroVec &operator=(const ZeroVec &) = delete;
  ~ZeroVec() { std::free(p); }
  void assign(size_t count, T zero) {
    (void)zero;
    std::free(p);
    p = count ? static_cast<T *>(std::calloc(count, sizeof(T))) : nullptr;
    n = p ? count : 0;
    if (count && !p) throw std::bad_alloc();
  }
  size_t size() const { return n; }
  bool empty() const { return n == 0; }
  T *data() { return p; }
  const T *data() const { return p; }
  T &operator[](size_t i) { return p[i]; }
  const T &operator[](size_t i) const { return p[i]; }
  const T *begin() const { return p; }
  const T *end() const { return p + n; }
};

struct EdgeStore {
  struct View {
    const int *p;
    size_t n;
    size_t size() const { return n; }
    bool empty() const { return n == 0; }
    const int *data() const { return p; }
    int operator[](size_t i) const { return p[i]; }
  };
  ZeroVec<long long> off;
  ZeroVec<int> cnt;
  std::vector<int> pool;
  void reset(long long G) { off.assign((size_t)G, 0); cnt.assign((size_t)G, 0); pool.clear(); }
  View operator[](long long g) const { return View{pool.data() + off[(size_t)g], (size_t)cnt[(size_t)g]}; }
  void set(long long g, const int *first, const int *last) {
    off[(size_t)g] = (long long)pool.size();
    cnt[(size_t)g] = (int)(last - first);
    pool.insert(pool.end(), first, last);
  }
};

struct TrackStore {
  std::vector<long long> off{0};
  std::vector<double> line7;
  std::vector<int> img_ids, line_ids, node_ids;
  std::vector<double> scores;
  std::vector<long long> gnodes;
  size_t size() const { return off.size() - 1; }
  size_t members() const { return img_ids.size(); }
  void clear() {
    off.assign(1, 0);
    line7.clear(); img_ids.clear(); line_ids.clear(); node_ids.clear(); scores.clear(); gnodes.clear();
  }
};

}

using lt_host::DevBuf;
using lt_host::TrackStore;

struct lt_ctx {
  using Cand = lt::Cand;
  lt_config cfg;
  int device = 0;
  hipStream_t stream = nullptr;
  bool own_stream = true;
  hipStream_t pool_stream = nullptr;
  std::string err;
  bool ranges_on = false;
  double lo[3] = {0, 0, 0}, hi[3] = {0, 0, 0};

  bool inited = false;
  int n_img = 0;
  std::vector<int> img_ids;
  std::unordered_map<int, int> id2idx;
  std::vector<long long> seg_off;
  long long G = 0;
  std::vector<int> h_node_img;
  std::vector<lt::Cam> h_cams;
  std::vector<double> h_segs;
  const double *h_segs_ptr = nullptr;
  double h_segs_add = 0.0;
  DevBuf d_kvec, d_qvec, d_tvec, d_segs_raw, d_cams, d_segs, d_seg_off, d_node_img;

  int job_mode = 0;
  std::vector<int> job_imgs;
  std::vector<std::vector<int>> job_nbs;
  std::vector<std::vector<int>> job_order;
  std::vector<long long> h_m_off;
  lt_host::RawInts h_m_pairs;
  size_t streamed_ints = 0;
  std::vector<long long> h_c_off, h_ovf_off;
  std::vector<int> h_line0;
  std::vector<unsigned> h_ovf;
  std::mutex ovf_mu;
  DevBuf d_c_stream, d_ovf, d_rowdesc;
  std::vector<char> triangulated;
  bool uploaded = false, ran = false, downloaded = false;
  std::vector<std::vector<int>> neighbors;

  int n_blk = 0;
  int max_nb = 1;
  long long P = 0;
  long long max_rows = 0;
  long long n_conn = 0;
  std::vector<long long> h_nb_off;
  std::vector<int> h_blk_img, h_blk_nb, h_blk_slot, h_blk_order;
  std::vector<long long> h_item_off;
  DevBuf d_nb_off, d_blk_img, d_blk_nb, d_blk_slot, d_blk_order, d_m_off, d_m_pairs, d_pairs;
  DevBuf d_keys, d_rows, d_row_blk, d_skeys, d_srows, d_sort_tmp, d_conn_off;
  DevBuf d_st_c, d_st_l, d_flags, d_pos, d_scan_tmp;
  DevBuf d_item_off, d_masks, d_mask_cnt, d_mask_pos;
  DevBuf d_rm_line, d_rm_act, d_rm_edges, d_rm_cnt;
  std::vector<unsigned long long> h_rm_edges;
  std::vector<unsigned long long> h_rm_back;
  std::vector<double> h_rm_in;
  DevBuf d_hcand, d_hlite;
  DevBuf d_cand, d_lite, d_tri_off, d_score, d_best_idx, d_edge_flag, d_nvalid, d_edge_off, d_edges;
  DevBuf d_best_c, d_best_score, d_best_src, d_ntris, d_err;
  DevBuf d_blk_line_base, d_cnt_bl, d_st_key, d_wave_count, d_wave_pos, d_ntris_u, d_cand_node, d_pair_counter;
  int max_own_segs = 0;
  int max_nb_segs = 0;
  long long stat_pairs_eval = 0;
  std::vector<long long> h_blk_line_base;
  bool rows_sorted = true;
  bool rows_ln = false;
  int ln_slots = 0;
  DevBuf d_run_len, d_slot_row0, d_blk_nruns, d_ln_flag;
  DevBuf d_blk_surv, d_blk_rnd0, d_round_count;
  long long n_round_slots = 0;
  lt_host::HostBlock h_pinned_blk;
  long long *h_pinned = nullptr;
  DevBuf d_chunks, d_cand_meta, d_st_row, d_surv_count, d_seg_gates, d_blkrec, d_seg_vp, d_seg_has_vp;
  DevBuf d_needed;
  int n_needed = 0;
  long long max_needed_segs = 0;
  DevBuf d_blk_chunk_off;
  int max_chunks = 1;
  DevBuf d_perm, d_rng;
  DevBuf d_result3;
  DevBuf d_scan_status;
  DevBuf d_tile_order;
  DevBuf d_tile_list;
  DevBuf d_blk_vorder;
  bool blk_vorder_ok = false;
  DevBuf d_pc_cnt, d_pc_list;
  DevBuf d_sp_slots, d_sp_cnt, d_sp_ovf, d_sp_pairs, d_sp_desc;
  bool score_two_kernels = false;
  bool score_fused = false;
  DevBuf d_base_bl;
  DevBuf d_place_perm;
  bool perm_mode = false;
  DevBuf d_ex_rec;
  DevBuf d_node_rec;
  DevBuf d_ex_ent;
  DevBuf d_ex_z;
  long long ex_region_cap = 0;
  double ex_frac = 0.0;
  bool ex_two_pass = false;
  bool ex_staged_set[2] = {false, false};
  bool in_run_async = false;
  bool pend_fine_gen = false, pend_fine_score = false;
  int ex_retry_depth = 0;
  bool host_view_valid = false;
  bool compact_valid = false;
  DevBuf d_tail_keys, d_tail_skeys, d_tail_sims, d_tail_mark, d_tail_pos, d_tail_recs, d_tail_nodes, d_tail_tmp, d_tail_keep, d_tail_kpos;
  bool cnt_bl_clean = false;
  size_t cnt_bl_bytes = 0;
  std::vector<double> h_seg_pts, h_sfm_xyz;
  std::vector<long long> h_seg_pt_off;
  std::vector<int> h_sfm_ids;
  DevBuf d_seg_pts, d_seg_pt_off, d_sfm_xyz;
  bool pts_ready = false, sfm_given = false, pts_dirty = false;
  long long max_seg_pts = 0;
  bool vp_ready = false;
  int n_chunks = 0;
  long long cand_cap = 0;
  long long C = 0, E = 0;
  long long shard_keys = -1, shard_keys_cap = 0, shard_own_keys = -1;

  lt_host::HostBlock best_c_blk;
  lt_host::HostBlock init_blk;
  Cand *best_c = nullptr;
  std::vector<char> best_c_set;
  lt_host::ZeroVec<double> best_score;
  lt_host::ZeroVec<int> best_src2, n_tris;
  lt_host::ZeroVec<unsigned char> has_best;
  lt_host::EdgeStore valid_edges;
  struct DebugTri {
    double line10[10], score;
    int src2[2];
  };
  std::vector<DebugTri> dbg_pool;
  lt_host::ZeroVec<long long> dbg_off;
  lt_host::ZeroVec<int> dbg_cnt;
  TrackStore tracks;
  struct GEdge {
    double sim;
    int n1, n2;
  };
  struct TailPending {
    bool active = false;
    long long E = 0;
    lt_host::HostBlock hb;
    size_t max_nodes = 0, o_pairs = 0, o_recs = 0, o_nodes = 0, o_flags = 0;
    int kb = 0;
    bool filtered = false;
  } tail_pend;
  DevBuf d_outer_flags;
  hipEvent_t ev_tail = nullptr;
  std::vector<int> tail_gmap;
  std::vector<int> tail_kmap;
  std::vector<long long> tail_gnode;
  std::vector<GEdge> tail_ge, tail_ge2;
  std::vector<int> tail_img_tmp;
  std::vector<int> tail_parent, tail_img_cnt, tail_labels, tail_nimg, tail_img_arena, tail_set_len;
  std::vector<long long> tail_set_off;
  std::vector<double> tail_cscore;
  std::vector<lt::Cand> tail_ccand;
  std::vector<unsigned char> valid_flags;
  bool tracks_done = false;
  long long stat_graph_nodes = 0, stat_graph_edges = 0, stat_pairs = 0;
  double timers[24] = {0};
  double timer_sums[24] = {0};
  long long timer_runs = 0;
  long long stat_survivors = 0;
  hipEvent_t ev[14] = {nullptr};
  hipEvent_t ev_b[14] = {nullptr};
  hipEvent_t ev_end[3] = {nullptr};
  unsigned run_seq = 0;
  hipEvent_t pend_ev_start = nullptr, pend_ev_end = nullptr;
  unsigned async_seq = 0;
  bool pend_sampled = true;
  long long timer_stage_runs = 0;
  bool run_pending = false;
  int pend_set = 0;
  bool pend_count_on_device = false;
  long long pend_C = 0;
  int pend_ev_gen_end = 3, pend_ev_place_end = 4;
  long long C_last = 0;
  std::vector<int> mg_node_img, mg_node_line;
  std::vector<int> mg_e1, mg_e2;
  std::vector<double> mg_sim;
  double mg_timers[4] = {0, 0, 0, 0};
  DevBuf d_mg_lines, d_mg_blks, d_mg_edges;
  double ft_timers[4] = {0, 0, 0, 0};
  DevBuf d_ft_maps, d_ft_imgs, d_ft_in, d_ft_out, d_ft_scr;
  double ev_timers[4] = {0, 0, 0, 0};
  DevBuf d_ev_in, d_ev_lines, d_ev_th, d_ev_out, d_ev_cnt;
  double bp_timers[4] = {0, 0, 0, 0};
  std::vector<long long> bp_edge_off;
  std::vector<int> bp_edge;
  std::vector<long long> bp_junc_off, bp_jid_off;
  std::vector<double> bp_junc_xy;
  std::vector<int> bp_jid;
  std::vector<long long> bp_cand_off;
  std::vector<double> bp_cand_xy;
  std::vector<int> bp_cand_lines, bp_parents;
  DevBuf d_bp_raw, d_bp_lines, d_bp_pts, d_bp_off, d_bp_off2, d_bp_off3, d_bp_blk, d_bp_cnt, d_bp_scan, d_bp_out,
      d_bp_inter, d_bp_cand, d_bp_keys, d_bp_keys2, d_bp_idx, d_bp_idx2, d_bp_tmp, d_bp_misc;
  double mt_timers[4] = {0, 0, 0, 0};
  std::vector<long long> mt_row_off, mt_slot_off;
  std::vector<int> mt_kk;
  std::vector<unsigned short> mt_col;
  std::vector<float> mt_score;
  bool mt_mutual = false;
  DevBuf d_mt_desc, d_mt_tasks, d_mt_units, d_mt_col, d_mt_score, d_mt_flag;
  double vp_timers[6] = {0, 0, 0, 0, 0, 0};
  std::vector<int> vp_labels, vp_clusters;
  std::vector<long long> vp_vp_off;
  std::vector<double> vp_vps;
  DevBuf d_vp_raw, d_vp_flag, d_vp_src, d_vp_lines, d_vp_imgs, d_vp_blk, d_vp_hyp, d_vp_pref, d_vp_state, d_vp_roots;

  double rf_timers[4] = {0, 0, 0, 0};
  std::vector<double> rf_out;
  DevBuf d_rf_k, d_rf_q, d_rf_t, d_rf_cam, d_rf_l2d, d_rf_l3d, d_rf_tab, d_rf_line, d_rf_tracks, d_rf_out;
};

#define HIPCHK(ctx, call)                                                                  \
  do {                                                                                     \
    hipError_t e_ = (call);                                                                \
    if (e_ != hipSuccess) {                                                                \
      (ctx)->err = std::string("HIP error: ") + hipGetErrorString(e_) + " at " #call;      \
      return LT_ERR_HIP;                                                                   \
    }                                                                                      \
  } while (0)

#define ENSURE(ctx, buf, bytes)                                                 \
  do {                                                                          \
    if (!(buf).ensure(bytes)) {                                                 \
      (ctx)->err = "hipMalloc failed for " #buf;                                \
      return LT_ERR_HIP;                                                        \
    }                                                                           \
  } while (0)

static inline int fail(lt_ctx *ctx, int code, const std::string &msg) {
  ctx->err = msg;
  return code;
}

namespace lt_impl {
int refine_with_ctx_cams(lt_ctx *ctx, int64_t n_tracks, const double *line6, const int64_t *off, const int32_t *img,
                         const double *line2d4, const double *line3d6, const lt_refine_config *cfg);
}
```

### limap_amd/csrc/lt_host.h

```cpp
#pragma once

#include "lt_ctx.h"
#include "lt_tail.h"
#include "lt_rows.h"
#include "lt_pool.h"

#include <algorithm>
#include <atomic>
#include <parallel/algorithm>
#include <chrono>
#include <cmath>
#include <cstdio>
#include <cstring>
#include <dlfcn.h>
#include <map>
#include <mutex>
#include <queue>
#include <set>
#include <string>
#include <unordered_map>
#include <vector>

namespace lt {
void launch_fn_query(hipStream_t st, const double *in30, int by_endpoints, double *out32);
int gen_slots(long long max_rows);
int gen_groups(long long max_rows);
int gen_slots_ln(int max_own_segs);
int gen_max_run();
void launch_rows_ln(hipStream_t st, int n_blk, int n_slots, const void *desc, const unsigned *stream,
                    const long long *blk_line_base, unsigned *rstart, int *blk_nruns, unsigned *run_len,
                    unsigned *slot_row0, unsigned short *tr, int *ln_flag);
size_t seg_gate_bytes();
void launch_build_blk(hipStream_t st, int n_blk, const long long *m_off, const int *blk_img, const int *blk_nb,
                      const int *blk_slot, const long long *seg_off, const long long *blk_line_base, void *blkrec);
size_t blk_rec_bytes();
void launch_gen_split(hipStream_t st, int n_blk, long long max_rows, const GenCfg &cfg, const long long *m_off,
                      const int *m_pairs, const int *blk_img, const int *blk_nb, const int *blk_slot,
                      const long long *seg_off, const Cam *cams, const Seg *segs, const PairRec *pairs,
                      const long long *blk_line_base, CRec *st_r, double *st_unc, unsigned *st_key,
                      unsigned *wave_count, unsigned *cnt_bl, int lds_segs, int lds_segs1, void *st_row,
                      unsigned *surv_count, long long n_segs, void *gates, void *blkrec, hipEvent_t *ev3,
                      const double *seg_vp, const unsigned char *seg_has_vp, const long long *seg_pt_off,
                      const void *seg_pts, const double *sfm_xyz, int *err_flag, int many_on, int one_on,
                      const long long *group_base, int phase, int ln_slots, const unsigned short *tr,
                      const unsigned *run_len, const unsigned *slot_row0, unsigned *blk_surv, const unsigned *blk_rnd0,
                      unsigned *round_count, const int *blk_vorder, unsigned *tri_unit_ctr);
size_t seg_point_bytes();
void launch_node_prefix(hipStream_t st, long long G, const int *node_img, const long long *seg_off,
                        const long long *nb_off, const long long *blk_line_base, unsigned *cnt_bl,
                        unsigned *base_bl, unsigned *n_tris, long long *tri_off, unsigned long long *status,
                        int *err_flag, void *node_rec);
void launch_expand_rows(hipStream_t st, int n_blk, const void *desc, const unsigned *stream, const unsigned *ovf, unsigned *rows);
void launch_place(hipStream_t st, int n_blk, long long max_rows, const long long *m_off, const int *blk_img,
                  const long long *seg_off, const long long *blk_line_base, const unsigned *base_bl,
                  const unsigned *wave_count, const long long *tri_off, const CRec *st_r, const double *st_unc,
                  const unsigned *st_key, CRec *cand, double *cand_unc, unsigned *cand_node, const long long *group_base,
                  unsigned *perm, const unsigned *blk_surv, const unsigned *blk_rnd0, const unsigned *round_count);
void launch_pack_keys(hipStream_t st, int n_blk, long long max_rows, const long long *m_off,
                      const unsigned *wave_count, const long long *wave_pos, const unsigned *st_key,
                      unsigned *keys_c, unsigned *src_c, const long long *group_base);
void launch_permute(hipStream_t st, long long C, const unsigned *skeys, const unsigned *ssrc, const CRec *st_r,
                    const double *st_unc, CRec *cand, double *cand_unc, unsigned *cand_node);
void launch_host_view(hipStream_t st, long long C, const unsigned *perm, const CRec *rec, const double *unc, Cand *out_c,
                      CandLite *out_l);
void launch_cand_node(hipStream_t st, long long G, const long long *tri_off, unsigned *cand_node);
size_t score3_lds_bytes(int max_nb, bool f32);
size_t cand_meta_bytes();
void launch_score3(hipStream_t st, long long C, long long G, const long long *tri_off, const unsigned *cand_node,
                   void *meta, const CRec *cand, const int *node_img, const long long *nb_off,
                   const int *blk_order, const Cam *cams, double *score, unsigned long long *pair_counter,
                   int max_nb, const ScoreCfg &cfg, double scaleinv_guard2, hipEvent_t ev_before, unsigned *draw,
                   bool f32, unsigned *perm, void *rng, bool perm_is_placement, unsigned *bucket_cnt,
                   unsigned *bucket_list, unsigned bucket_cap, const unsigned *place, unsigned *rec, const float *st_z,
                   int *err_flag, void *sp_slots, int sp_slot_cap, unsigned *sp_cnt, unsigned *sp_ovf, void *sp_pairs,
                   void *sp_desc, long long sp_chunks, hipEvent_t ev_after, const void *node_rec, unsigned *pc_cnt,
                   void *pc_list, unsigned pc_cap, int one_kernel);
size_t score_split_chunk_bytes();
size_t score_split_entry_bytes();
long long score_split_chunks(long long C);
int score3_tile_buckets();
}

namespace lt_trace {
struct Range {
  bool on;
  explicit Range(const char *name);
  ~Range();
};
}
#define LT_CONCAT2(a, b) a##b
#define LT_CONCAT(a, b) LT_CONCAT2(a, b)
#define LT_RANGE(name) lt_trace::Range LT_CONCAT(lt_range_, __LINE__)(name)

namespace lt_impl {
const char *test_switch(const char *name);
int fine_level();
bool fine_timers();
bool fine_gen_timers();
double now_ms();
double multiplier(double score_th);
lt::LinkCfg2 make_l2(const lt_config &c);
lt::LinkCfg3 make_l3(const lt_config &c);
lt::GenCfg make_gen(const lt_ctx *ctx);
lt::ScoreCfg make_score(const lt_ctx *ctx);
int bits_for(long long n);
void build_job_tables(lt_ctx *ctx);
int upload_points(lt_ctx *ctx);
int finish_run(lt_ctx *ctx);
void define_best_of_other_images(lt_ctx *ctx);
int materialize_compact(lt_ctx *ctx);

template <class T>
int upload_vec(lt_ctx *ctx, DevBuf &buf, const std::vector<T> &v) {
  ENSURE(ctx, buf, sizeof(T) * std::max<size_t>(v.size(), 1));
  if (!v.empty())
    HIPCHK(ctx, hipMemcpyAsync(buf.p, v.data(), sizeof(T) * v.size(), hipMemcpyHostToDevice, ctx->stream));
  return LT_OK;
}
}

#define LT_FINISH(ctx)                       \
  do {                                       \
    int rc_fin_ = lt_impl::finish_run(ctx);  \
    if (rc_fin_) return rc_fin_;             \
  } while (0)
```

### limap_amd/csrc/lt_kernels_v2.hip

```cpp

#include "lt_devfn.h"

#include <algorithm>

namespace lt {

#ifndef LT_GEN_CHUNKS
#define LT_GEN_CHUNKS 5
#endif
#ifndef LT_GATE_WAVES
#define LT_GATE_WAVES 8
#endif
#ifndef LT_GATE_WAVES_PER_EU
#define LT_GATE_WAVES_PER_EU 4
#endif
#define LT_GATE_OCC __attribute__((amdgpu_waves_per_eu(LT_GATE_WAVES_PER_EU, LT_GATE_WAVES_PER_EU)))
constexpr int kGenChunks = LT_GEN_CHUNKS;
constexpr int kRowsPerWave = 64 * kGenChunks;
constexpr int kGateWaves = LT_GATE_WAVES;
#ifndef LT_TRI_SLOTS
#define LT_TRI_SLOTS 4
#endif
constexpr int kTriSlots = LT_TRI_SLOTS;
#ifndef LT_TRI_WAVES
// ... 912 lines not shown
    unsigned pos32 = 0;
    if (act) {
      const unsigned rank = (unsigned)(lane - my_head) + (my_head == 0 ? carry : 0u);
      const long long pos = tri_off[key] + base_bl[lbase + (long long)(key - g1)] + rank;
      pos32 = (unsigned)pos;
      cand_node[pos] = key;
      if (perm) perm[pos] = (unsigned)(s0 + lane);
    }
    if (perm) continue;
    const double2 *src_c = reinterpret_cast<const double2 *>(st_r + s0);
    double2 *dst_c = reinterpret_cast<double2 *>(cand);
#pragma unroll
    for (int it = 0; it < 8; ++it) {
      const unsigned u = (unsigned)it * 64u + (unsigned)lane;
      const unsigned ci = u >> 3, piece = u & 7u;
      const unsigned p = (unsigned)__shfl((int)pos32, (int)ci);
      if (u < count * 8u) dst_c[(size_t)p * 8u + piece] = src_c[u];
    }
    if (act) cand_unc[pos32] = st_unc[s0 + lane];
  }
  }
}

__global__ void __launch_bounds__(256)
k_node_prefix(long long G, const int *__restrict__ node_img, const long long *__restrict__ seg_off,
              const long long *__restrict__ nb_off, const long long *__restrict__ blk_line_base,
              unsigned *__restrict__ cnt_bl, unsigned *__restrict__ base_bl, unsigned *__restrict__ n_tris,
              long long *__restrict__ tri_off, unsigned long long *__restrict__ status, int *__restrict__ err_flag,
              uint4 *__restrict__ node_rec) {
  __shared__ unsigned s_tile;
  __shared__ long long s_wave[4];
  __shared__ long long s_prefix;
  if (threadIdx.x == 0) s_tile = (unsigned)atomicAdd(&status[0], 1ull);
  __syncthreads();
  const long long tile = s_tile;
  const long long g = tile * 256 + threadIdx.x;
  const int lane = lane_id(), wave = threadIdx.x >> 6;
  unsigned run = 0;
  unsigned nbv = 0;
  if (g < G) {
    int img = node_img[g];
    int line = (int)(g - seg_off[img]);
    const long long b0 = nb_off[img], b1 = nb_off[img + 1];
    nbv = ((unsigned)b0 << 8) | (unsigned)(b1 - b0);
    for (long long bb = b0; bb < b1; bb += 16) {
      long long e[16];
      unsigned c[16];
#pragma unroll
      for (int k = 0; k < 16; ++k) {
        e[k] = (bb + k < b1) ? blk_line_base[bb + k] + line : -1;
      }
#pragma unroll
      for (int k = 0; k < 16; ++k) c[k] = e[k] >= 0 ? cnt_bl[e[k]] : 0u;
#pragma unroll
      for (int k = 0; k < 16; ++k) {
        if (e[k] >= 0) {
          cnt_bl[e[k]] = 0;
          base_bl[e[k]] = run;
        }
        run += c[k];
      }
    }
  }
  long long incl = (long long)run;
#pragma unroll
  for (int d = 1; d < 64; d <<= 1) {
    const long long o = __shfl_up(incl, d);
    if (lane >= d) incl += o;
  }
  if (lane == 63) s_wave[wave] = incl;
  __syncthreads();
  long long wbase = 0;
  for (int w = 0; w < wave; ++w) wbase += s_wave[w];
  const long long total = s_wave[0] + s_wave[1] + s_wave[2] + s_wave[3];
  constexpr unsigned long long kMask = (1ull << 62) - 1ull;
  if (wave == 0) {
    long long prefix = 0;
    if (tile > 0) {
      if (lane == 0) atomicExch(&status[1 + tile], (1ull << 62) | (unsigned long long)total);
      long long hi = tile;
      bool done = false;
      while (!done) {
        const long long k = hi - 1 - lane;
        unsigned long long v = 2ull << 62;
        if (k >= 0) {
          int budget = 1 << 22;
          do {
            v = atomicAdd(&status[1 + k], 0ull);
          } while ((v >> 62) == 0ull && --budget > 0);
          if ((v >> 62) == 0ull) {
            *err_flag = 4;
            v = 2ull << 62;
          }
        }
        const unsigned long long incl_lanes = __ballot((v >> 62) == 2ull);
        const int first = incl_lanes ? __builtin_ctzll(incl_lanes) : 64;
        long long part = (lane <= first) ? (long long)(v & kMask) : 0ll;
        for (int d = 32; d >= 1; d >>= 1) part += __shfl_xor(part, d);
        prefix += part;
        if (first < 64) done = true;
        else hi -= 64;
      }
    }
    if (lane == 0) {
      atomicExch(&status[1 + tile], (2ull << 62) | (unsigned long long)(prefix + total));
      s_prefix = prefix;
    }
  }
  __syncthreads();
  const long long off = s_prefix + wbase + incl - (long long)run;
  if (g <= G) {
    tri_off[g] = off;
    n_tris[g] = run;
  }
  if (node_rec && g < G) node_rec[g] = uint4{(unsigned)(off & 0xFFFFFFFFll), (unsigned)(off >> 32), run, nbv};
}

template <int kTS>
__global__ void __launch_bounds__(256)
k_place(const long long *__restrict__ m_off, const int *__restrict__ blk_img,
        const long long *__restrict__ seg_off, const long long *__restrict__ blk_line_base,
        const unsigned *__restrict__ base_bl, const unsigned *__restrict__ wave_count,
        const long long *__restrict__ tri_off, const CRec *__restrict__ st_r,
        const double *__restrict__ st_unc, const unsigned *__restrict__ st_key, CRec *__restrict__ cand,
        double *__restrict__ cand_unc, unsigned *__restrict__ cand_node, int n_groups,
        const long long *__restrict__ group_base, unsigned *__restrict__ perm,
        const unsigned *__restrict__ slot_row0) {
  const int wave = threadIdx.x >> 6;
  const int lane = lane_id();
  const int b = blockIdx.y;
  const int g = blockIdx.x * 4 + wave;
  if (g >= n_groups) return;
  const int n_slots = n_groups * kTS;
  const long long rb = m_off[b], re = m_off[b + 1];
  const long long r0 = slot_first_row(slot_row0, n_slots, b, g * kTS, rb);
  if (r0 >= re) return;
  const unsigned lin = (unsigned)b * (unsigned)n_groups + (unsigned)g;
  const unsigned count = wave_count[lin];
  if (count == 0) return;
  const long long g1 = seg_off[blk_img[b]];
  const long long lbase = blk_line_base[b];
  const long long s0 = group_base ? group_base[lin] : r0;
  static_assert(sizeof(CRec) == 8 * 16, "record size in 16-byte units");
  for (unsigned e0 = 0; e0 < count; e0 += 64) {
    const unsigned e = e0 + lane;
    const bool act = e < count;
    unsigned pos32 = 0;
    const unsigned key = act ? st_key[s0 + e] : 0xFFFFFFFFu;
    const unsigned prev = (unsigned)__shfl_up((int)key, 1);
    const bool head = act && (lane == 0 || key != prev);
    const unsigned long long heads = __ballot(head);
    const int my_head = 63 - __builtin_clzll(heads & ((2ull << lane) - 1ull) | 1ull);
    const unsigned key0 = (unsigned)__builtin_amdgcn_readfirstlane((int)key);
    unsigned carry = 0;
    {
      long long cur_r0 = r0;
      int cur_g = g;
      long long idx_end = (long long)e0;
      unsigned cur_lin = lin;
      while (true) {
        bool more = true;
        while (idx_end > 0) {
          const long long j = idx_end - 64 + lane;
          const bool valid = j >= 0;
          const unsigned k = valid ? st_key[(group_base ? group_base[cur_lin] : cur_r0) + j] : 0u;
          const unsigned long long m = __ballot(valid && k == key0);
          const unsigned lead = m == ~0ull ? 64u : (unsigned)__builtin_clzll(~m);
          carry += lead;
          const long long n_valid = idx_end < 64 ? idx_end : 64;
          if ((long long)lead < n_valid) { more = false; break; }
          idx_end -= n_valid;
        }
        if (!more) break;
        if (cur_g == 0) break;
        cur_g -= 1;
        cur_r0 = slot_first_row(slot_row0, n_slots, b, cur_g * kTS, rb);
        cur_lin -= 1;
        idx_end = (long long)wave_count[cur_lin];
      }
    }
    if (act) {
      const unsigned rank = (unsigned)(lane - my_head) + (my_head == 0 ? carry : 0u);
      const long long toff = tri_off[key];
      const long long pos = toff + base_bl[lbase + (long long)(key - g1)] + rank;
      pos32 = (unsigned)pos;
      cand_node[pos] = key;
      if (perm) perm[pos] = (unsigned)(s0 + e);
    }
    if (perm) continue;
    const unsigned nb = min(64u, count - e0);
    const double2 *src_c = reinterpret_cast<const double2 *>(st_r + s0 + e0);
    double2 *dst_c = reinterpret_cast<double2 *>(cand);
#pragma unroll
    for (int it = 0; it < 8; ++it) {
      const unsigned u = (unsigned)it * 64u + (unsigned)lane;
      const unsigned ci = u >> 3, piece = u & 7u;
      const unsigned p = (unsigned)__shfl((int)pos32, (int)ci);
      if (u < nb * 8u) dst_c[(size_t)p * 8u + piece] = src_c[u];
    }
    if (act) cand_unc[pos32] = st_unc[s0 + e];
  }
}

__global__ void __launch_bounds__(256)
k_pack_keys(const long long *__restrict__ m_off, const unsigned *__restrict__ wave_count,
            const long long *__restrict__ wave_pos, const unsigned *__restrict__ st_key,
            unsigned *__restrict__ keys_c, unsigned *__restrict__ src_c, int n_groups,
            const long long *__restrict__ group_base) {
  const int wave = threadIdx.x >> 6;
  const int lane = lane_id();
  const int b = blockIdx.y;
  const int g = blockIdx.x * 4 + wave;
  if (g >= n_groups) return;
  const long long rb = m_off[b], re = m_off[b + 1];
  const long long r0 = rb + (long long)g * kTriRows;
  if (r0 >= re) return;
  const unsigned lin = (unsigned)b * (unsigned)n_groups + (unsigned)g;
  const unsigned count = wave_count[lin];
  const long long base = wave_pos[lin];
  for (unsigned e = lane; e < count; e += 64) {
    const long long s0 = group_base ? group_base[lin] : r0;
    keys_c[base + e] = st_key[s0 + e];
    src_c[base + e] = (unsigned)(s0 + e);
  }
}

__global__ void k_permute(long long C, const unsigned *__restrict__ skeys, const unsigned *__restrict__ ssrc,
                          const CRec *__restrict__ st_r, const double *__restrict__ st_unc,
                          CRec *__restrict__ cand, double *__restrict__ cand_unc, unsigned *__restrict__ cand_node) {
  long long t = (long long)blockIdx.x * blockDim.x + threadIdx.x;
  if (t >= C) return;
  unsigned src = ssrc[t];
  cand[t] = st_r[src];
  cand_unc[t] = st_unc[src];
  cand_node[t] = skeys[t];
}

__global__ void k_host_view(long long C, const unsigned *__restrict__ perm, const CRec *__restrict__ rec,
                            const double *__restrict__ unc, Cand *__restrict__ out_c, CandLite *__restrict__ out_l) {
  long long t = (long long)blockIdx.x * blockDim.x + threadIdx.x;
  if (t >= C) return;
  const long long src = perm ? (long long)perm[t] : t;
  Cand c;
  CandLite l;
  crec_split(rec[src], unc[src], &c, &l);
  out_c[t] = c;
  out_l[t] = l;
}

static inline unsigned nblk2(long long n, int bs) { return (unsigned)((n + bs - 1) / bs); }

int gen_slots(long long max_rows) {
  long long n = (max_rows + kRowsPerWave - 1) / kRowsPerWave;
  n = (n + kGateWaves - 1) / kGateWaves * kGateWaves;
  return (int)n;
}
int gen_groups(long long max_rows) { return gen_slots(max_rows) / kTriSlots; }
int gen_slots_ln(int max_own_segs) {
  int n = (max_own_segs + 63) / 64;
  return std::max((n + kGateWaves - 1) / kGateWaves * kGateWaves, kGateWaves);
}
int gen_max_run() { return kMaxRun; }
void launch_rows_ln(hipStream_t st, int n_blk, int n_slots, const void *desc, const unsigned *stream,
                    const long long *blk_line_base, unsigned *rstart, int *blk_nruns, unsigned *run_len,
                    unsigned *slot_row0, unsigned short *tr, int *ln_flag) {
  if (n_blk <= 0) return;
  hipLaunchKernelGGL(k_rows_starts, dim3((unsigned)n_blk), dim3(256), 0, st, n_blk, reinterpret_cast<const RowDesc *>(desc),
                     stream, blk_line_base, rstart, blk_nruns, ln_flag);
  hipLaunchKernelGGL(k_rows_transpose, dim3(nblk2(n_slots, 4), (unsigned)n_blk), dim3(256), 0, st, n_blk, n_slots,
                     reinterpret_cast<const RowDesc *>(desc), stream, blk_line_base, rstart, blk_nruns, run_len, slot_row0, tr,
                     ln_flag);
}
#ifdef LT_TRACE
int score_read_trace(unsigned long long *host, size_t n);
extern "C" int lt_debug_read_trace(unsigned long long *host, size_t n) {
  const int rc = (int)hipMemcpyFromSymbol(host, HIP_SYMBOL(g_trace), n * 8, 0, hipMemcpyDeviceToHost);
  return rc ? rc : score_read_trace(host, n);
}
#endif
size_t seg_gate_bytes() { return sizeof(SegGate); }
size_t seg_point_bytes() { return sizeof(SegPoint); }
size_t blk_rec_bytes() { return sizeof(BlkRec); }
void launch_expand_rows(hipStream_t st, int n_blk, const void *desc, const unsigned *stream, const unsigned *ovf, unsigned *rows) {
  if (n_blk > 0)
    hipLaunchKernelGGL(k_expand_rows, dim3((unsigned)n_blk), dim3(64 * kExpandWaves), 0, st, n_blk, reinterpret_cast<const RowDesc *>(desc), stream,
                       ovf, rows);
}
void launch_build_blk(hipStream_t st, int n_blk, const long long *m_off, const int *blk_img, const int *blk_nb,
                      const int *blk_slot, const long long *seg_off, const long long *blk_line_base, void *blkrec) {
  if (n_blk > 0)
    hipLaunchKernelGGL(k_build_blk, dim3(nblk2(n_blk, 128)), dim3(128), 0, st, n_blk, m_off, blk_img, blk_nb, blk_slot,
                       seg_off, blk_line_base, reinterpret_cast<BlkRec *>(blkrec));
}
void launch_gen_split(hipStream_t st, int n_blk, long long max_rows, const GenCfg &cfg, const long long *m_off,
                      const int *m_pairs, const int *blk_img, const int *blk_nb, const int *blk_slot,
                      const long long *seg_off, const Cam *cams, const Seg *segs, const PairRec *pairs,
                      const long long *blk_line_base, CRec *st_r, double *st_unc, unsigned *st_key,
                      unsigned *wave_count, unsigned *cnt_bl, int lds_segs, int lds_segs1, void *st_row,
                      unsigned *surv_count, long long n_segs, void *gates, void *blkrec, hipEvent_t *ev3,
                      const double *seg_vp, const unsigned char *seg_has_vp, const long long *seg_pt_off,
                      const void *seg_pts, const double *sfm_xyz, int *err_flag, int many_on, int one_on,
                      const long long *group_base, int phase, int ln_slots, const unsigned short *tr,
                      const unsigned *run_len, const unsigned *slot_row0, unsigned *blk_surv, const unsigned *blk_rnd0,
                      unsigned *round_count, const int *blk_vorder, unsigned *tri_unit_ctr) {
  if (n_blk <= 0 || max_rows <= 0) return;
  static int n_cu = 0;
  if (n_cu == 0) {
    int dev = 0;
    if (hipGetDevice(&dev) != hipSuccess ||
        hipDeviceGetAttribute(&n_cu, hipDeviceAttributeMultiprocessorCount, dev) != hipSuccess || n_cu <= 0)
      n_cu = 256;
  }
  GenArgs a;
  a.m_off = m_off; a.m_pairs = m_pairs; a.blk_img = blk_img; a.blk_nb = blk_nb; a.blk_slot = blk_slot;
  a.seg_off = seg_off; a.cams = cams; a.segs = segs; a.gates = reinterpret_cast<const SegGate *>(gates);
  a.pairs = pairs; a.blk_line_base = blk_line_base; a.st_row = reinterpret_cast<uint2 *>(st_row); a.surv_count = surv_count;
  a.st_r = st_r; a.st_unc = st_unc; a.st_key = st_key; a.wave_count = wave_count; a.cnt_bl = cnt_bl;
  const bool ln = ln_slots > 0;
  a.n_slots = ln ? ln_slots : gen_slots(max_rows); a.lds_segs = lds_segs; a.lds_segs1 = lds_segs1;
  a.tr = ln ? tr : nullptr; a.run_len = ln ? run_len : nullptr; a.slot_row0 = ln ? slot_row0 : nullptr;
  a.seg_vp = seg_vp; a.seg_has_vp = seg_has_vp;
  a.seg_pt_off = seg_pt_off; a.seg_pts = reinterpret_cast<const SegPoint *>(seg_pts); a.sfm_xyz = sfm_xyz;
  a.err_flag = err_flag;
  const bool extra = seg_vp || seg_pts;
  a.group_base = extra ? group_base : nullptr;
  a.count_only = (extra && phase == 1) ? 1 : 0;
  a.many_on = many_on; a.one_on = one_on;
  a.blk = reinterpret_cast<const BlkRec *>(blkrec); a.n_blk = n_blk;
  const bool ln_w4 = ln && (size_t)lds_segs * sizeof(SegGate) <= 40 * 1024;
  const int gate_waves = ln ? (ln_w4 ? 4 : 8) : kGateWaves;
  const long long n_items = (long long)n_blk * (a.n_slots / gate_waves);
  const size_t lds = ln ? (size_t)lds_segs * sizeof(SegGate) : (size_t)(lds_segs + lds_segs1) * sizeof(SegGate);
  int per_cu = std::max(16 / gate_waves, 1);
  if (lds > 0) per_cu = (int)std::max<size_t>(std::min<size_t>(160 * 1024 / lds, (size_t)per_cu), 1);
  const unsigned n_wg = (unsigned)std::min<long long>(n_items, (long long)n_cu * per_cu);
  const dim3 grid(n_wg), block(64 * gate_waves);
  if (ev3 && phase != 2) (void)hipEventRecord(ev3[0], st);
  if (phase != 2 && ln) {
    if (ln_w4)
      hipLaunchKernelGGL((k_gates_ln<4>), grid, block, lds, st, a, cfg, a.blk, a.pairs, a.tr, a.run_len, a.slot_row0, a.st_row,
                         blk_surv, blk_vorder);
    else
      hipLaunchKernelGGL((k_gates_ln<8>), grid, block, lds, st, a, cfg, a.blk, a.pairs, a.tr, a.run_len, a.slot_row0, a.st_row,
                         blk_surv, blk_vorder);
  } else if (phase != 2) {
    if (lds_segs1 > 0 && lds_segs > 0) hipLaunchKernelGGL((k_gates<true, true>), grid, block, lds, st, a, cfg, a.blk, a.pairs);
    else if (lds_segs > 0) hipLaunchKernelGGL((k_gates<false, true>), grid, block, lds, st, a, cfg, a.blk, a.pairs);
    else if (lds_segs1 > 0) hipLaunchKernelGGL((k_gates<true, false>), grid, block, lds, st, a, cfg, a.blk, a.pairs);
    else hipLaunchKernelGGL((k_gates<false, false>), grid, block, lds, st, a, cfg, a.blk, a.pairs);
  }
  if (ev3 && phase != 2) (void)hipEventRecord(ev3[1], st);
  const size_t tri_lds = kTriWaves * (64 * 9 + 16) * sizeof(double2);
  if (ln) {
    const dim3 tg((unsigned)std::min<long long>(n_blk, (long long)n_cu * (16 / kTriWaves)));
    hipLaunchKernelGGL(k_tri_rounds, tg, dim3(64 * kTriWaves), tri_lds, st, a, cfg, a.cams, a.pairs, a.blk, blk_surv, blk_rnd0,
                       round_count, blk_vorder, tri_unit_ctr);
  } else {
    const dim3 tg(nblk2(a.n_slots / kTriSlots, kTriWaves), n_blk);
    if (extra)
      hipLaunchKernelGGL((k_tri_rows<true, kTriSlots>), tg, dim3(64 * kTriWaves), 0, st, a, cfg, a.cams, a.pairs, a.blk, a.slot_row0);
    else
      hipLaunchKernelGGL((k_tri_rows<false, kTriSlots>), tg, dim3(64 * kTriWaves), tri_lds, st, a, cfg, a.cams, a.pairs, a.blk,
                         a.slot_row0);
  }
  if (ev3 && phase != 1) (void)hipEventRecord(ev3[2], st);
}
void launch_node_prefix(hipStream_t st, long long G, const int *node_img, const long long *seg_off,
                        const long long *nb_off, const long long *blk_line_base, unsigned *cnt_bl,
                        unsigned *base_bl, unsigned *n_tris, long long *tri_off, unsigned long long *status,
                        int *err_flag, void *node_rec) {
  hipLaunchKernelGGL(k_node_prefix, dim3(nblk2(G + 1, 256)), dim3(256), 0, st, G, node_img, seg_off, nb_off,
                     blk_line_base, cnt_bl, base_bl, n_tris, tri_off, status, err_flag, reinterpret_cast<uint4 *>(node_rec));
}
void launch_place(hipStream_t st, int n_blk, long long max_rows, const long long *m_off, const int *blk_img,
                  const long long *seg_off, const long long *blk_line_base, const unsigned *base_bl,
                  const unsigned *wave_count, const long long *tri_off, const CRec *st_r, const double *st_unc,
                  const unsigned *st_key, CRec *cand, double *cand_unc, unsigned *cand_node, const long long *group_base,
                  unsigned *perm, const unsigned *blk_surv, const unsigned *blk_rnd0, const unsigned *round_count) {
  if (n_blk <= 0 || max_rows <= 0) return;
  if (round_count) {
    static int n_cu = 0;
    if (n_cu == 0) {
      int dev = 0;
      if (hipGetDevice(&dev) != hipSuccess ||
          hipDeviceGetAttribute(&n_cu, hipDeviceAttributeMultiprocessorCount, dev) != hipSuccess || n_cu <= 0)
        n_cu = 256;
    }
    hipLaunchKernelGGL(k_place_rounds, dim3((unsigned)std::min<long long>(n_blk, (long long)n_cu * LT_PLACE_WG_PER_CU)), dim3(256), 0, st, m_off,
                       blk_img, seg_off, blk_line_base, base_bl, tri_off, st_r, st_unc, st_key, cand, cand_unc, cand_node, perm,
                       blk_surv, blk_rnd0, round_count, n_blk);
    return;
  }
  const int n_groups = gen_groups(max_rows);
  hipLaunchKernelGGL(k_place<kTriSlots>, dim3(nblk2(n_groups, 4), n_blk), dim3(256), 0, st, m_off, blk_img, seg_off,
                     blk_line_base, base_bl, wave_count, tri_off, st_r, st_unc, st_key, cand, cand_unc, cand_node, n_groups,
                     group_base, perm, (const unsigned *)nullptr);
}
void launch_pack_keys(hipStream_t st, int n_blk, long long max_rows, const long long *m_off,
                      const unsigned *wave_count, const long long *wave_pos, const unsigned *st_key,
                      unsigned *keys_c, unsigned *src_c, const long long *group_base) {
  if (n_blk <= 0 || max_rows <= 0) return;
  const int n_groups = gen_groups(max_rows);
  hipLaunchKernelGGL(k_pack_keys, dim3(nblk2(n_groups, 4), n_blk), dim3(256), 0, st, m_off, wave_count, wave_pos,
                     st_key, keys_c, src_c, n_groups, group_base);
}
void launch_permute(hipStream_t st, long long C, const unsigned *skeys, const unsigned *ssrc, const CRec *st_r,
                    const double *st_unc, CRec *cand, double *cand_unc, unsigned *cand_node) {
  if (C > 0)
    hipLaunchKernelGGL(k_permute, dim3(nblk2(C, 256)), dim3(256), 0, st, C, skeys, ssrc, st_r, st_unc, cand, cand_unc,
                       cand_node);
}
void launch_host_view(hipStream_t st, long long C, const unsigned *perm, const CRec *rec, const double *unc, Cand *out_c,
                      CandLite *out_l) {
  if (C > 0) hipLaunchKernelGGL(k_host_view, dim3(nblk2(C, 256)), dim3(256), 0, st, C, perm, rec, unc, out_c, out_l);
}
}
```

Baseline: 2.510 billion.

## Run selection kernel on a side stream to overlap with next run's gate stage

```diff
diff --git a/limap_amd/csrc/lt_api.cpp b/limap_amd/csrc/lt_api.cpp
--- a/limap_amd/csrc/lt_api.cpp
+++ b/limap_amd/csrc/lt_api.cpp
@@ -530,6 +530,11 @@
   (void)finish_run(ctx);
   (void)hipSetDevice(ctx->device);
   (void)hipStreamSynchronize(ctx->stream);
+  if (ctx->side_stream) {
+    (void)hipStreamSynchronize(ctx->side_stream);
+    (void)hipStreamDestroy(ctx->side_stream);
+    ctx->side_stream = nullptr;
+  }
   DevBuf *bufs[] = {&ctx->d_kvec, &ctx->d_qvec, &ctx->d_tvec, &ctx->d_segs_raw, &ctx->d_cams, &ctx->d_segs,
                     &ctx->d_seg_off, &ctx->d_node_img, &ctx->d_nb_off, &ctx->d_blk_img, &ctx->d_blk_nb,
                     &ctx->d_blk_slot, &ctx->d_blk_order, &ctx->d_m_off, &ctx->d_m_pairs, &ctx->d_c_stream, &ctx->d_ovf, &ctx->d_rowdesc, &ctx->d_pairs,
@@ -571,6 +576,11 @@
 int lt_set_stream(lt_ctx *ctx, void *hip_stream) {
   LT_FINISH(ctx);
   HIPCHK(ctx, hipStreamSynchronize(ctx->stream));
+  if (ctx->side_stream) {
+    HIPCHK(ctx, hipStreamSynchronize(ctx->side_stream));
+    HIPCHK(ctx, hipStreamDestroy(ctx->side_stream));
+    ctx->side_stream = nullptr;
+  }
   if (hip_stream) {
     ctx->stream = reinterpret_cast<hipStream_t>(hip_stream);
     ctx->own_stream = false;
diff --git a/limap_amd/csrc/lt_api_run.cpp b/limap_amd/csrc/lt_api_run.cpp
--- a/limap_amd/csrc/lt_api_run.cpp
+++ b/limap_amd/csrc/lt_api_run.cpp
@@ -181,12 +181,12 @@
     ctx->C_last = ctx->pend_count_on_device ? hp[0] : ctx->pend_C;
   } else {
     HIPCHK(ctx, hipStreamSynchronize(ctx->stream));
-    HIPCHK(ctx, hipMemcpy(&derr, ctx->d_err.p, sizeof(int), hipMemcpyDeviceToHost));
+    HIPCHK(ctx, hipMemcpy(&derr, ctx->d_err.as<int>() + 32 * ctx->pend_set, sizeof(int), hipMemcpyDeviceToHost));
     unsigned long long pe = 0;
     ctx->C_last = ctx->pend_C;
     if (ctx->pend_count_on_device)
       HIPCHK(ctx, hipMemcpy(&ctx->C_last, ctx->d_tri_off.as<long long>() + ctx->G, 8, hipMemcpyDeviceToHost));
-    if (ctx->C_last > 0) HIPCHK(ctx, hipMemcpy(&pe, ctx->d_pair_counter.p, 8, hipMemcpyDeviceToHost));
+    if (ctx->C_last > 0) HIPCHK(ctx, hipMemcpy(&pe, ctx->d_pair_counter.as<unsigned long long>() + 16 * ctx->pend_set, 8, hipMemcpyDeviceToHost));
     ctx->stat_pairs_eval = (long long)pe;
   }
   ctx->stat_survivors = -1;
@@ -279,7 +279,11 @@
 }
 }
 }
-int lt_sync(lt_ctx *ctx) { return finish_run(ctx); }
+int lt_sync(lt_ctx *ctx) {
+  const int rc = finish_run(ctx);
+  if (ctx->side_stream && hipStreamSynchronize(ctx->side_stream) != hipSuccess && !rc) return fail(ctx, LT_ERR_HIP, "HIP error: synchronising the side stream");
+  return rc;
+}
 
 int lt_run_device_async(lt_ctx *ctx) {
   LT_RANGE("lt_run_device (enqueue: generation, placement, scoring, selection)");
@@ -310,6 +314,29 @@
   HIPCHK(ctx, hipSetDevice(ctx->device));
   hipStream_t st = ctx->stream;
   const long long G = ctx->G, P = ctx->P;
+  constexpr long long kCountFreeBytes = 48ll << 30;
+  const long long per_cand = (!test_switch("LT_TEST_PLACE_COPY") ? 4 : (long long)(sizeof(CRec) + 8)) + 8 + 4 + 4 +
+                             (long long)cand_meta_bytes() + (long long)score_split_entry_bytes() * 256 / 64;
+  const bool count_free = ctx->h_pinned && P * per_cand <= kCountFreeBytes && !test_switch("LT_TEST_SYNC_COUNT");
+  const bool vp_now = ctx->cfg.use_vp && !ctx->cfg.disable_vp_triangulation;
+  const bool pts_now = ctx->pts_ready && (!ctx->cfg.disable_many_points_triangulation || !ctx->cfg.disable_one_point_triangulation);
+  const bool extras_now = vp_now || pts_now;
+  const bool select_side = hp && ctx->run_pending && ctx->pend_ev_end && ctx->job_mode == 1 && ctx->rows_ln && ctx->rows_sorted &&
+                           !extras_now && count_free && G > 0 && P > 0 && ctx->n_blk > 0 && ctx->max_rows > 0 &&
+                           !test_switch("LT_TEST_SELECT_MAIN_STREAM");
+  if (select_side && !ctx->side_stream) {
+    int prio = 0;
+    if (hipStreamGetPriority(st, &prio) != hipSuccess) {
+      (void)hipGetLastError();
+      prio = 0;
+    }
+    HIPCHK(ctx, hipStreamCreateWithPriority(&ctx->side_stream, hipStreamNonBlocking, prio));
+  }
+  hipEvent_t wait_prev_select = (ctx->run_pending && ctx->pend_select_side) ? ctx->pend_ev_end : nullptr;
+  if (wait_prev_select && !select_side) {
+    HIPCHK(ctx, hipStreamWaitEvent(st, wait_prev_select, 0));
+    wait_prev_select = nullptr;
+  }
   {
     int rcp = upload_points(ctx);
     if (rcp) return rcp;
@@ -322,8 +349,10 @@
   const bool guards_on = scfg.l3.th_scaleinv > 0.0 && scfg.l3.score_th > 0.0 && scfg.l3.score_th < 1.0 &&
                          !test_switch("LT_TEST_NO_SCORE_GUARDS");
   const double guard2 = guards_on ? (scfg.l3.th_scaleinv * (1.0 + 1e-6)) * (scfg.l3.th_scaleinv * (1.0 + 1e-6)) : 1e300;
-  ENSURE(ctx, ctx->d_err, sizeof(int));
-  ENSURE(ctx, ctx->d_pair_counter, 8);
+  ENSURE(ctx, ctx->d_err, 256);
+  ENSURE(ctx, ctx->d_pair_counter, 256);
+  int *const d_err = ctx->d_err.as<int>() + 32 * set;
+  unsigned long long *const d_pair_counter = ctx->d_pair_counter.as<unsigned long long>() + 16 * set;
   ENSURE(ctx, ctx->d_result3, 32);
   ENSURE(ctx, ctx->d_pairs, sizeof(PairRec) * (size_t)std::max(ctx->n_blk, 1));
   ENSURE(ctx, ctx->d_tri_off, sizeof(long long) * (size_t)(G + 1));
@@ -336,8 +365,8 @@
   const bool ln_job = ctx->job_mode == 1 && ctx->rows_ln && ctx->rows_sorted;
   if (ln_job) ENSURE(ctx, ctx->d_blk_surv, 4 * (size_t)std::max(ctx->n_blk, 1));
   launch_build_pairs(st, ctx->n_blk, ctx->d_blk_img.as<int>(), ctx->d_blk_nb.as<int>(), ctx->d_cams.as<Cam>(),
-                     ctx->d_pairs.as<PairRec>(), ctx->d_err.as<int>(),
-                     ctx->d_pair_counter.as<unsigned long long>(), ctx->d_scan_status.as<unsigned long long>(),
+                     ctx->d_pairs.as<PairRec>(), d_err,
+                     d_pair_counter, ctx->d_scan_status.as<unsigned long long>(),
                      n_status, ln_job ? ctx->d_blk_surv.as<unsigned>() : nullptr);
 
   bool node_rec_valid = false;
@@ -349,9 +378,7 @@
     const size_t Pn = (size_t)std::max<long long>(P, 1);
     const bool fast = ctx->rows_sorted;
     {
-      const bool vp_now = ctx->cfg.use_vp && !ctx->cfg.disable_vp_triangulation;
-      const bool pts_now = ctx->pts_ready && (!ctx->cfg.disable_many_points_triangulation || !ctx->cfg.disable_one_point_triangulation);
-      if (ctx->rows_ln && (vp_now || pts_now)) {
+      if (ctx->rows_ln && extras_now) {
         launch_expand_rows(st, ctx->n_blk, ctx->d_rowdesc.p, ctx->d_c_stream.as<unsigned>(), ctx->d_ovf.as<unsigned>(),
                            ctx->d_m_pairs.as<unsigned>());
         ctx->rows_ln = false;
@@ -363,9 +390,9 @@
     const long long n_waves = (long long)ctx->n_blk * gen_groups(ctx->max_rows);
     const long long n_slots_all = (long long)ctx->n_blk * (ln ? ln_slots : gen_slots(ctx->max_rows));
     const long long n_entries = ctx->h_blk_line_base[ctx->n_blk];
-    const bool vp_on = ctx->cfg.use_vp && !ctx->cfg.disable_vp_triangulation;
+    const bool vp_on = vp_now;
     if (vp_on && !ctx->vp_ready) return fail(ctx, LT_ERR_STATE, "use_vp is set but InitVPResults was not called");
-    const bool pts_any = ctx->pts_ready && (!ctx->cfg.disable_many_points_triangulation || !ctx->cfg.disable_one_point_triangulation);
+    const bool pts_any = pts_now;
     const bool many_on = pts_any && !ctx->cfg.disable_many_points_triangulation;
     const bool one_on = pts_any && !ctx->cfg.disable_one_point_triangulation;
     const bool pts_on = pts_any;
@@ -413,13 +440,15 @@
                        vp_on ? ctx->d_seg_vp.as<double>() : nullptr,
                        vp_on ? ctx->d_seg_has_vp.as<unsigned char>() : nullptr,
                        pts_on ? ctx->d_seg_pt_off.as<long long>() : nullptr, pts_on ? ctx->d_seg_pts.p : nullptr,
-                       (pts_on && ctx->sfm_given) ? ctx->d_sfm_xyz.as<double>() : nullptr, ctx->d_err.as<int>(),
+                       (pts_on && ctx->sfm_given) ? ctx->d_sfm_xyz.as<double>() : nullptr, d_err,
                        many_on ? 1 : 0, one_on ? 1 : 0, group_base, phase, ln_slots, ctx->d_m_pairs.as<unsigned short>(),
                        ctx->d_run_len.as<unsigned>(), ctx->d_slot_row0.as<unsigned>(), ctx->d_blk_surv.as<unsigned>(),
                        ctx->d_blk_rnd0.as<unsigned>(), ctx->d_round_count.as<unsigned>(),
                        (ctx->blk_vorder_ok && !test_switch("LT_TEST_GATES_IMAGE_MAJOR")) ? ctx->d_blk_vorder.as<int>() : nullptr,
                        test_switch("LT_TEST_TRI_STATIC") ? nullptr
-                           : (unsigned *)(ctx->d_scan_status.as<unsigned long long>() + n_status_scan + score3_tile_buckets() * 16 + ex_regions() * 16));
+                           : (unsigned *)(ctx->d_scan_status.as<unsigned long long>() + n_status_scan + score3_tile_buckets() * 16 + ex_regions() * 16),
+                       wait_prev_select);
+      wait_prev_select = nullptr;
       };
       if (!extras) {
         gen(0);
@@ -441,6 +470,7 @@
         gen(2);
       }
     }
+    if (wait_prev_select) return fail(ctx, LT_ERR_RUNTIME, "internal: the wait for the previous run's k_select was not enqueued");
     bool gen_event_pending = false;
     if (fine_gen && ctx->n_blk > 0 && ctx->max_rows > 0) ev_gen_end = 10;
     else gen_event_pending = true;
@@ -453,17 +483,13 @@
                          ctx->d_nb_off.as<long long>(), ctx->d_blk_line_base.as<long long>(),
                          ctx->d_cnt_bl.as<unsigned>(), ctx->d_base_bl.as<unsigned>(), ctx->d_ntris_u.as<unsigned>(),
                          ctx->d_tri_off.as<long long>(), ctx->d_scan_status.as<unsigned long long>(),
-                         ctx->d_err.as<int>(), ctx->d_node_rec.p);
+                         d_err, ctx->d_node_rec.p);
       node_rec_valid = true;
       ctx->cnt_bl_clean = true;
       const long long bound = P;
-      constexpr long long kCountFreeBytes = 48ll << 30;
-      const bool perm_bound = !test_switch("LT_TEST_PLACE_COPY");
-      const long long per_cand = (perm_bound ? 4 : (long long)(sizeof(CRec) + 8)) + 8 + 4 + 4 + (long long)cand_meta_bytes() +
-                                 (long long)score_split_entry_bytes() * 256 / 64;
       if (extras) {
         C_known = staged_total;
-      } else if (ctx->h_pinned && bound * per_cand <= kCountFreeBytes && !test_switch("LT_TEST_SYNC_COUNT")) {
+      } else if (count_free) {
         C_known = -1;
         C_bound = bound;
       } else {
@@ -542,12 +568,12 @@
     ctx->perm_mode = false;
     ctx->compact_valid = true;
     const size_t In = (size_t)std::max<long long>(P, 1);
-    const bool vp_on = ctx->cfg.use_vp && !ctx->cfg.disable_vp_triangulation;
+    const bool vp_on = vp_now;
     if (vp_on && !ctx->vp_ready) return fail(ctx, LT_ERR_STATE, "use_vp is set but InitVPResults was not called");
     const double *seg_vp = vp_on ? ctx->d_seg_vp.as<double>() : nullptr;
     const unsigned char *seg_has_vp = vp_on ? ctx->d_seg_has_vp.as<unsigned char>() : nullptr;
     const int n_masks = vp_on ? 3 : 1;
-    const bool pts_any = ctx->pts_ready && (!ctx->cfg.disable_many_points_triangulation || !ctx->cfg.disable_one_point_triangulation);
+    const bool pts_any = pts_now;
     const int many_on = (pts_any && !ctx->cfg.disable_many_points_triangulation) ? 1 : 0;
     const int one_on = (pts_any && !ctx->cfg.disable_one_point_triangulation) ? 1 : 0;
     const double *sfm_xyz = (pts_any && ctx->sfm_given) ? ctx->d_sfm_xyz.as<double>() : nullptr;
@@ -592,7 +618,7 @@
                                 ctx->d_cams.as<Cam>(), ctx->d_segs.as<Seg>(), ctx->d_pairs.as<PairRec>(),
                                 ctx->d_masks.as<unsigned short>(), ctx->d_mask_cnt.as<unsigned>(), nullptr, nullptr,
                                 nullptr, seg_vp, seg_has_vp, ctx->d_seg_pt_off.as<long long>(), ctx->d_seg_pts.p,
-                                sfm_xyz, ctx->d_err.as<int>(), many_on, one_on, ctx->d_blk_chunk_off.as<int>(),
+                                sfm_xyz, d_err, many_on, one_on, ctx->d_blk_chunk_off.as<int>(),
                                 ctx->max_nb, ctx->max_chunks, ctx->d_seg_gates.p);
     } else {
       if (plain && !test_switch("LT_TEST_EX_PASS1_BLOCK"))
@@ -601,7 +627,7 @@
                                 ctx->d_cams.as<Cam>(), ctx->d_segs.as<Seg>(), ctx->d_pairs.as<PairRec>(),
                                 ctx->d_masks.as<unsigned long long>(), ctx->d_blk_chunk_off.as<int>(), ctx->d_seg_gates.p,
                                 staged ? ctx->d_ex_ent.as<unsigned long long>() : nullptr, ex_ctr, region_cap,
-                                ctx->d_err.as<int>());
+                                d_err);
       else
       launch_gen_exhaustive(st, false, P, gcfg, ctx->d_item_off.as<long long>(), G, ctx->d_node_img.as<int>(),
                             ctx->d_nb_off.as<long long>(), ctx->d_blk_nb.as<int>(), ctx->d_seg_off.as<long long>(),
@@ -636,7 +662,7 @@
     }
     if (staged) {
       launch_tri_offsets_ex(st, G, ctx->d_item_off.as<long long>(), ctx->d_mask_pos.as<long long>(), P, -1, ex_cap,
-                            ctx->d_tri_off.as<long long>(), ctx->d_err.as<int>());
+                            ctx->d_tri_off.as<long long>(), d_err);
       if (sampled) HIPCHK(ctx, hipEventRecord(ev[3], st));
       launch_place_exhaustive(st, ex_ctr, region_cap, ctx->d_ex_ent.as<unsigned long long>(),
                               ctx->d_st_key.as<unsigned>(), ctx->d_item_off.as<long long>(),
@@ -667,7 +693,7 @@
                                 ctx->d_masks.as<unsigned short>(), ctx->d_mask_cnt.as<unsigned>(),
                                 ctx->d_mask_pos.as<long long>(), ctx->d_cand.as<CRec>(), ctx->d_lite.as<double>(),
                                 seg_vp, seg_has_vp, ctx->d_seg_pt_off.as<long long>(), ctx->d_seg_pts.p, sfm_xyz,
-                                ctx->d_err.as<int>(), many_on, one_on, ctx->d_blk_chunk_off.as<int>(), ctx->max_nb,
+                                d_err, many_on, one_on, ctx->d_blk_chunk_off.as<int>(), ctx->max_nb,
                                 ctx->max_chunks, ctx->d_seg_gates.p);
     else if (!vp_on && !test_switch("LT_TEST_EX_PASS2_BLOCK"))
       launch_fill_exhaustive(st, ctx->n_blk, P, gcfg, ctx->d_item_off.as<long long>(), ctx->d_blk_img.as<int>(),
@@ -683,7 +709,7 @@
                             ctx->d_cand.as<CRec>(), ctx->d_lite.as<double>(), seg_vp, seg_has_vp,
                             ctx->d_blk_chunk_off.as<int>(), ctx->max_nb, ctx->max_chunks, ctx->d_seg_gates.p);
     launch_tri_offsets_ex(st, G, ctx->d_item_off.as<long long>(), ctx->d_mask_pos.as<long long>(), P, total, -1,
-                          ctx->d_tri_off.as<long long>(), ctx->d_err.as<int>());
+                          ctx->d_tri_off.as<long long>(), d_err);
     ENSURE(ctx, ctx->d_cand_node, 4 * Cn);
     launch_cand_node(st, G, ctx->d_tri_off.as<long long>(), ctx->d_cand_node.as<unsigned>());
     C_known = total;
@@ -742,7 +768,7 @@
     launch_score3(st, C_bound, G, ctx->d_tri_off.as<long long>(), ctx->d_cand_node.as<unsigned>(), ctx->d_cand_meta.p,
                   ctx->perm_mode ? ctx->d_st_c.as<CRec>() : ctx->d_cand.as<CRec>(), ctx->d_node_img.as<int>(),
                   ctx->d_nb_off.as<long long>(), ctx->d_blk_order.as<int>(), ctx->d_cams.as<Cam>(),
-                  ctx->d_score.as<double>(), ctx->d_pair_counter.as<unsigned long long>(), ctx->max_nb, scfg,
+                  ctx->d_score.as<double>(), d_pair_counter, ctx->max_nb, scfg,
                   guard2, fine_score ? ev[11] : nullptr, ctx->d_tile_order.as<unsigned>(), score_f32,
                   (ctx->perm_mode && !staged_sorted) ? ctx->d_place_perm.as<unsigned>()
                                                      : (score_sorted ? ctx->d_perm.as<unsigned>() : nullptr),
@@ -751,15 +777,16 @@
                   tile_classes ? ctx->d_tile_list.as<unsigned>() : nullptr, tile_cap,
                   staged_sorted ? ctx->d_place_perm.as<unsigned>() : nullptr,
                   staged_sorted ? ctx->d_ex_rec.as<unsigned>() : nullptr,
-                  staged_sorted ? ctx->d_ex_z.as<float>() : nullptr, ctx->d_err.as<int>(),
+                  staged_sorted ? ctx->d_ex_z.as<float>() : nullptr, d_err,
                   split ? ctx->d_sp_slots.p : nullptr, sp_slot_cap, ctx->d_sp_cnt.as<unsigned>(),
-                  ctx->d_sp_ovf.as<unsigned>(), ctx->d_sp_pairs.p, ctx->d_sp_desc.p, sp_chunks, sampled ? ev[5] : nullptr,
+                  ctx->d_sp_ovf.as<unsigned>(), ctx->d_sp_pairs.p, ctx->d_sp_desc.p, sp_chunks,
+                  (sampled || select_side) ? ev[5] : nullptr,
                   node_rec_valid ? ctx->d_node_rec.p : nullptr, pair_classes ? ctx->d_pc_cnt.as<unsigned>() : nullptr,
                   pair_classes ? ctx->d_pc_list.p : nullptr, tile_cap,
                   (((ctx->score_two_kernels || test_switch("LT_SCORE_TWO_KERNELS") || ctx->n_img >= (1 << 18))
                         ? 0 : (test_switch("LT_TEST_Q_LOSE_TILE") ? 2 : 1)) |
                    (test_switch("LT_TEST_DENSE_TABLES") ? 4 : 0) | (test_switch("LT_TEST_DENSE_FEW_ROWS") ? 8 : 0)));
-    if (C_bound <= 0 && sampled) HIPCHK(ctx, hipEventRecord(ev[5], st));
+    if (C_bound <= 0 && (sampled || select_side)) HIPCHK(ctx, hipEventRecord(ev[5], st));
   }
   ENSURE(ctx, ctx->d_best_idx, 8 * (size_t)std::max<long long>(G, 1));
   ENSURE(ctx, ctx->d_nvalid, 4 * (size_t)(G + 1));
@@ -768,13 +795,18 @@
   ENSURE(ctx, ctx->d_best_score, 8 * (size_t)std::max<long long>(G, 1));
   ENSURE(ctx, ctx->d_best_src, 8 * (size_t)std::max<long long>(G, 1));
   ENSURE(ctx, ctx->d_ntris, 4 * (size_t)std::max<long long>(G, 1));
-  launch_select(st, G, ctx->d_tri_off.as<long long>(), ctx->d_score.as<double>(), scfg.fullscore_th,
+  hipStream_t st_sel = st;
+  if (select_side) {
+    HIPCHK(ctx, hipStreamWaitEvent(ctx->side_stream, ev[5], 0));
+    st_sel = ctx->side_stream;
+  }
+  launch_select(st_sel, G, ctx->d_tri_off.as<long long>(), ctx->d_score.as<double>(), scfg.fullscore_th,
                 scfg.max_valid_conns, ctx->d_best_idx.as<long long>(), ctx->d_edge_flag.as<unsigned>(),
                 ctx->d_nvalid.as<unsigned>(), ctx->perm_mode ? ctx->d_st_c.as<CRec>() : ctx->d_cand.as<CRec>(),
                 ctx->perm_mode ? ctx->d_st_l.as<double>() : ctx->d_lite.as<double>(),
                 ctx->d_best_c.as<Cand>(), ctx->d_best_score.as<double>(), ctx->d_best_src.as<int>(),
-                ctx->d_ntris.as<int>(), ctx->job_mode == 2, ctx->d_err.as<int>(),
-                ctx->d_pair_counter.as<unsigned long long>(), hp ? hp : ctx->d_result3.as<long long>(),
+                ctx->d_ntris.as<int>(), ctx->job_mode == 2, d_err,
+                d_pair_counter, hp ? hp : ctx->d_result3.as<long long>(),
                 ctx->perm_mode ? ctx->d_place_perm.as<unsigned>() : nullptr);
   if (!hp) HIPCHK(ctx, hipEventRecord(ev[7], st));
   HIPCHK(ctx, hipGetLastError());
@@ -783,7 +815,7 @@
     if (!ctx->ev_end[0])
       for (auto &e : ctx->ev_end) HIPCHK(ctx, hipEventCreate(&e));
     ev_end = ctx->ev_end[ctx->run_seq++ % 3u];
-    HIPCHK(ctx, hipEventRecord(ev_end, st));
+    HIPCHK(ctx, hipEventRecord(ev_end, st_sel));
   }
   int rc_prev = LT_OK;
   if (ctx->run_pending) {
@@ -795,6 +827,7 @@
   ctx->pend_ev_start = ev_start;
   ctx->pend_sampled = sampled;
   ctx->pend_ev_end = ev_end;
+  ctx->pend_select_side = select_side;
   ctx->pend_set = set;
   ctx->pend_count_on_device = C_known < 0;
   ctx->pend_fine_gen = fine_gen;
diff --git a/limap_amd/csrc/lt_ctx.h b/limap_amd/csrc/lt_ctx.h
--- a/limap_amd/csrc/lt_ctx.h
+++ b/limap_amd/csrc/lt_ctx.h
@@ -326,6 +326,8 @@
   hipEvent_t ev_end[3] = {nullptr};
   unsigned run_seq = 0;
   hipEvent_t pend_ev_start = nullptr, pend_ev_end = nullptr;
+  hipStream_t side_stream = nullptr;
+  bool pend_select_side = false;
   unsigned async_seq = 0;
   bool pend_sampled = true;
   long long timer_stage_runs = 0;
diff --git a/limap_amd/csrc/lt_host.h b/limap_amd/csrc/lt_host.h
--- a/limap_amd/csrc/lt_host.h
+++ b/limap_amd/csrc/lt_host.h
@@ -44,7 +44,8 @@
                       const void *seg_pts, const double *sfm_xyz, int *err_flag, int many_on, int one_on,
                       const long long *group_base, int phase, int ln_slots, const unsigned short *tr,
                       const unsigned *run_len, const unsigned *slot_row0, unsigned *blk_surv, const unsigned *blk_rnd0,
-                      unsigned *round_count, const int *blk_vorder, unsigned *tri_unit_ctr);
+                      unsigned *round_count, const int *blk_vorder, unsigned *tri_unit_ctr,
+                      hipEvent_t wait_tri = nullptr);
 size_t seg_point_bytes();
 void launch_node_prefix(hipStream_t st, long long G, const int *node_img, const long long *seg_off,
                         const long long *nb_off, const long long *blk_line_base, unsigned *cnt_bl,
diff --git a/limap_amd/csrc/lt_kernels_v2.hip b/limap_amd/csrc/lt_kernels_v2.hip
--- a/limap_amd/csrc/lt_kernels_v2.hip
+++ b/limap_amd/csrc/lt_kernels_v2.hip
@@ -1238,7 +1238,8 @@
                       const void *seg_pts, const double *sfm_xyz, int *err_flag, int many_on, int one_on,
                       const long long *group_base, int phase, int ln_slots, const unsigned short *tr,
                       const unsigned *run_len, const unsigned *slot_row0, unsigned *blk_surv, const unsigned *blk_rnd0,
-                      unsigned *round_count, const int *blk_vorder, unsigned *tri_unit_ctr) {
+                      unsigned *round_count, const int *blk_vorder, unsigned *tri_unit_ctr,
+                      hipEvent_t wait_tri) {
   if (n_blk <= 0 || max_rows <= 0) return;
   static int n_cu = 0;
   if (n_cu == 0) {
@@ -1286,6 +1287,7 @@
     else hipLaunchKernelGGL((k_gates<false, false>), grid, block, lds, st, a, cfg, a.blk, a.pairs);
   }
   if (ev3 && phase != 2) (void)hipEventRecord(ev3[1], st);
+  if (wait_tri) (void)hipStreamWaitEvent(st, wait_tri, 0);
   const size_t tri_lds = kTriWaves * (64 * 9 + 16) * sizeof(double2);
   if (ln) {
     const dim3 tg((unsigned)std::min<long long>(n_blk, (long long)n_cu * (16 / kTriWaves)));
```

Result: faster. 2.549 billion, median of 6 (+1.6%).
